# Coder-Yu/SELFRec

Hardware: AMD Instinct MI355X
Metric: train pairs/sec (XSimGCL, Yelp2018-shape) (higher is better)
Workload: dtype f32; 1 GPU; XSimGCL L=3 l*=1 eps=0.2 lambda=0.2 tau=0.2, synthetic yelp2018-shape graph (31668 users x 38048 items, 1260793 train edges), d=64, B=2048, Adam lr=1e-3; global_batch=2048, parallelism=single, bit_reproducible_step=True, launch=hipGraph replay, epoch_boundaries_in_region=1, nce_products=f32 MFMA (v_mfma_f32_16x16x4_f32)

## Files before the change

### include/selfrec_hip.h

```cpp
#ifndef SELFREC_HIP_H
#define SELFREC_HIP_H

#include <stdint.h>

#ifdef __cplusplus
extern "C" {
#endif

typedef int32_t srh_status_t;
enum {
  SRH_OK = 0,
  SRH_ERR_INVALID_ARG = -1,
  SRH_ERR_HIP = -2,
  SRH_ERR_UNSUPPORTED = -3,
  SRH_ERR_NOMEM = -4,
  SRH_ERR_STATE = -5
};

#define SRH_ABI_VERSION 31
int32_t srh_abi_version(void);
const char* srh_last_error_string(void);
int32_t srh_device_count(void);

typedef struct srh_sampler srh_sampler_t;
// ... 18 lines not shown
                                        const int32_t* h_j, const int32_t* h_uniq_u, const int32_t* h_n_uniq_u,
                                        const int32_t* h_uniq_i, const int32_t* h_n_uniq_i, int32_t user_row0,
                                        int32_t item_row0, int32_t* h_n_uniq_n, int32_t* h_seg_rows, int32_t* h_seg_end,
                                        int32_t* h_seg, int32_t* h_seg_a, int32_t* h_seg_b);
srh_status_t srh_sampler_sample_range(srh_sampler_t* s, int64_t n, int64_t k, int64_t* h_out);
srh_status_t srh_sampler_next_u32(srh_sampler_t* s, uint32_t* out);

srh_status_t srh_find_k_largest_host(int64_t k, const float* h_candidates, int64_t n, int64_t* h_out_ids,
                                     float* h_out_scores, int64_t* out_count);

srh_status_t srh_find_k_largest_host_f64(int64_t k, const double* h_candidates, int64_t n, int64_t* h_out_ids,
                                         double* h_out_scores, int64_t* out_count);

srh_status_t srh_mt19937_uniform_f32(uint32_t* h_mt624, int32_t* pos, int64_t n, float* h_out,
                                     float keep_addend, uint8_t* h_keep);

srh_status_t srh_adj_sym_normalize(int64_t n_rows, const int32_t* d_indptr,
                                   const int32_t* d_indices, const int32_t* d_edge_id,
                                   const float* d_weight, const uint8_t* d_keep,
                                   const float* d_inv_sqrt_table, int32_t table_len,
                                   float* d_deg_ws, float* d_vals, int64_t row_offset, int32_t phase,
                                   void* stream);

typedef struct srh_spmm_plan srh_spmm_plan_t;

srh_status_t srh_spmm_plan_create(srh_spmm_plan_t** out, int64_t n_rows, int64_t n_cols,
                                  const int32_t* h_indptr, int32_t split_len ,
                                  int64_t xcd_split_row, const int32_t* h_row_mid);

srh_status_t srh_spmm_plan_set_xcd_shares(srh_spmm_plan_t* plan, int32_t d, const int32_t* h_blocks_per_xcd);
int32_t srh_spmm_plan_run_tasks(const srh_spmm_plan_t* plan, int32_t d);
void srh_spmm_plan_destroy(srh_spmm_plan_t* plan);

enum { SRH_EPI_PERTURB = 1, SRH_EPI_MEAN = 2, SRH_EPI_AXPY = 4, SRH_EPI_ADAM = 8 };
#define SRH_MAX_ADAM_CLEAR 4
#define SRH_MAX_PREV 8
#define SRH_MAX_ADD 2
#define SRH_MAX_EXTRA 2

typedef struct srh_spmm_epilogue {
  int32_t flags;
  float eps;
  const float* d_noise;
  uint64_t rng_seed;
  uint64_t rng_offset;
  const int64_t* d_rng_step;
  uint64_t rng_stride;
  int32_t n_prev;
  int32_t n_add;
  const float* d_prev[SRH_MAX_PREV];
  float mean_div;
  float alpha;
  float* d_mean_out;
  const float* d_add[SRH_MAX_ADD];
  float add_scale[SRH_MAX_ADD];
  const int32_t* d_row_mark;
  const int32_t* d_col_mark;
  const int64_t* d_mark_stamp;
  const int32_t* d_add_mark;
  int32_t add_sparse_mask;
  int32_t n_extra;
  int32_t main_clean;
  float* d_extra_out[SRH_MAX_EXTRA];
  const float* d_extra_noise[SRH_MAX_EXTRA];
  uint64_t extra_rng_offset[SRH_MAX_EXTRA];
  int32_t noise_d_full;
  int32_t noise_col0;
  const float* d_row_scale;
  int32_t scale_flags;
  int32_t prev_unscale_mask;
  int32_t add_rowscale_mask;
  int32_t noise_d_valid;
  float* d_adam_param;
  float* d_adam_m;
  float* d_adam_v;
  const float* d_adam_coef;
  float adam_beta1, adam_beta2, adam_eps;
  int32_t adam_n_clear;
  const int32_t* d_adam_clear_mark;
  float* d_adam_clear[SRH_MAX_ADAM_CLEAR];
  int64_t* d_adam_cursor;
} srh_spmm_epilogue_t;
enum { SRH_SCALE_IN = 1, SRH_SCALE_OUT = 2 };

srh_status_t srh_spmm_f32(const srh_spmm_plan_t* plan, const int32_t* d_indptr,
                          const int32_t* d_indices, const float* d_vals, const float* d_x,
                          float* d_y, int32_t d, const srh_spmm_epilogue_t* epi, void* stream);

srh_status_t srh_spmm3_f32(const srh_spmm_plan_t* plan, const int32_t* d_indices, const float* d_vals0,
                           const float* d_vals1, const float* d_vals2, const float* d_x, float* d_y0,
                           float* d_y1, float* d_y2, int32_t d, void* stream);

typedef struct srh_batch_segments {
  const int32_t* d_n_uniq_u;
  const int32_t* d_n_uniq_i;
  const int32_t* d_n_uniq_n;
  const int32_t* d_seg_rows;
  const int32_t* d_seg_end;
  const int32_t* d_seg;
  const int32_t* d_seg_a;
  const int32_t* d_seg_b;
  const int32_t* d_batch_no;
  int32_t nce_rows;
  int32_t rows_are_zero;
} srh_batch_segments_t;
int64_t srh_bpr_ws_bytes(int64_t B);
srh_status_t srh_bpr_l2_fwd_bwd(const float* d_user, const float* d_item,
                                const float* d_reg_user, const float* d_reg_item,
                                const int32_t* d_u_idx, const int32_t* d_i_idx,
                                const int32_t* d_j_idx, int64_t B, const int32_t* d_n_rows,
                                int32_t d, float reg_coef, int32_t reg_include_neg,
                                float loss_scale, float* d_g_user, float* d_g_item,
                                float* d_greg_user, float* d_greg_item, double* d_losses,
                                void* d_ws, void* stream);
// ... 33 lines not shown
  int32_t g2_exclusive;
} srh_infonce_problem_t;
srh_status_t srh_infonce_fwd_bwd_multi(const srh_infonce_problem_t* problems, int32_t n_problems,
                                       int32_t d, float tau, float loss_scale, double* d_loss,
                                       void* d_ws, int32_t precision, void* stream);

#define SRH_NCE_SPLIT16 0
#define SRH_NCE_SPLIT_BF16 SRH_NCE_SPLIT16
#define SRH_NCE_F32 1
#define SRH_NCE_DEFAULT (-1)
srh_status_t srh_infonce_set_precision(int32_t mode);
int32_t srh_infonce_get_precision(void);

typedef struct srh_bpr_problem {
  const float* d_user;
  const float* d_item;
  const float* d_reg_user;
  const float* d_reg_item;
  const int32_t* d_u_idx;
  const int32_t* d_i_idx;
  const int32_t* d_j_idx;
  int64_t B;
  const int32_t* d_n_rows;
  float reg_coef;
  int32_t reg_include_neg;
  float loss_scale;
  float* d_g_user;
  float* d_g_item;
  float* d_greg_user;
  float* d_greg_item;
  double* d_losses;
  void* d_ws;
  const srh_batch_segments_t* seg;
} srh_bpr_problem_t;
srh_status_t srh_bpr_l2_fwd_bwd_p(const srh_bpr_problem_t* bpr, int32_t d, void* stream);
srh_status_t srh_bpr_infonce_fwd_bwd(const srh_bpr_problem_t* bpr, const srh_infonce_problem_t* problems,
                                     int32_t n_problems, int32_t d, float tau, float cl_scale,
                                     double* d_cl_loss, void* d_nce_ws, int32_t precision, void* stream);

srh_status_t srh_adam_step(float* d_param, const float* d_grad, float* d_m, float* d_v,
                           int64_t n_elem, int64_t step, const int64_t* d_step, float lr,
                           float beta1, float beta2, float eps, void* stream);
srh_status_t srh_adam_step_reset(float* d_param, const float* d_grad, float* d_m, float* d_v, int64_t n_rows,
                                 int32_t d, const int64_t* d_step, float lr, float beta1, float beta2, float eps,
                                 const int32_t* d_row_mark, int32_t n_clear, float* const* d_clear_tables,
                                 int64_t* d_cursor_advance, void* stream);

srh_status_t srh_score_mask_topk(const float* d_user_emb, const int32_t* d_user_ids,
                                 int64_t n_query, const float* d_item_emb, int64_t n_items,
                                 int32_t d, const int32_t* d_r_indptr, const int32_t* d_r_indices,
                                 int32_t k, float* d_scores_ws, int64_t ws_rows, int32_t* d_out_ids,
                                 float* d_out_scores, void* stream);
int64_t srh_score_mask_topk_filtered_ws_bytes(int64_t chunk_rows, int64_t sample_items, int32_t k, int32_t cap,
                                              int64_t n_items, int32_t d);
srh_status_t srh_score_mask_topk_filtered(const float* d_user_emb, const int32_t* d_user_ids, int64_t n_query,
                                          const float* d_item_emb, int64_t n_items, int32_t d,
                                          const int32_t* d_r_indptr, const int32_t* d_r_indices, int32_t k,
                                          int64_t sample_items, int32_t cap, int64_t chunk_rows, void* d_ws,
                                          int32_t* d_out_ids, float* d_out_scores, int32_t* d_out_counts,
                                          void* stream);
srh_status_t srh_topk_trim_mark_ties(const int32_t* d_ids, const float* d_scores, int64_t n_query, int32_t k1,
                                     int32_t* d_out_ids, float* d_out_scores, void* stream);
srh_status_t srh_gemm_nt_f32(const float* d_a, const float* d_b, float* d_c, int64_t m,
                             int64_t n, int32_t d, void* stream);
srh_status_t srh_topk_rows(const float* d_scores, int64_t rows, int64_t n, int32_t k,
                           int32_t* d_out_ids, float* d_out_scores, void* stream);
// ... 3 lines not shown
                                const int32_t* d_t_indices, uint8_t* d_flags, void* stream);
srh_status_t srh_metric_rows(const uint8_t* d_flags, const int32_t* d_sizes, int64_t n_query, int32_t k,
                             const int32_t* cuts, int32_t n_cuts, const double* d_gains, const double* d_ideal,
                             int32_t* d_hits, double* d_ndcg, void* stream);

srh_status_t srh_axpby(float a, const float* d_x, float b, float* d_y, int64_t n_elem, void* stream);
typedef struct {
  const int32_t* d_epoch_u;
  const int32_t* d_epoch_i;
  const int32_t* d_epoch_j;
  const int32_t* d_epoch_uniq_u;
  const int32_t* d_epoch_uniq_i;
  const int32_t* d_n_uniq_u;
  const int32_t* d_n_uniq_i;
  int64_t n_edges;
  int64_t batch_size;
  const int64_t* d_cursor;
  int32_t* d_stage_u;
  int32_t* d_stage_i;
  int32_t* d_stage_j;
  int32_t* d_stage_uniq_u;
  int32_t* d_stage_uniq_i;
  int32_t* d_meta;
  int32_t* d_row_mark;
  int32_t mark_item_offset;
  int32_t cat_item_offset;
  double* d_zero4;
  int32_t* d_stage_cat;
  int32_t* d_n_cat;
  int64_t* d_now;
  int64_t half_batches;
  float* d_adam_coef;
  float adam_lr, adam_beta1, adam_beta2;
} srh_batch_fetch_args_t;
srh_status_t srh_batch_fetch(const srh_batch_fetch_args_t* args, void* stream);
srh_status_t srh_spmm_f32_with_fetch(const srh_spmm_plan_t* plan, const int32_t* d_indptr, const int32_t* d_indices,
                                     const float* d_vals, const float* d_x, float* d_y, int32_t d,
                                     const srh_spmm_epilogue_t* epi, const srh_batch_fetch_args_t* fetch, void* stream);

srh_status_t srh_spmm_f32_probe(const srh_spmm_plan_t* plan, const int32_t* d_indices, const float* d_vals,
                                const float* d_x, float* d_y, int32_t d, const srh_spmm_epilogue_t* epi,
                                uint64_t* d_stamps, void* stream);
srh_status_t srh_spmm_gather_bound(const srh_spmm_plan_t* plan, const int32_t* d_indices, const float* d_x, float* d_scratch,
                                   int32_t d, void* stream);
srh_status_t srh_gather_floor_probe(const int32_t* d_indices, int64_t n_idx, const float* d_x, int64_t n_x_rows, int32_t d,
                                    int32_t blocks, float* d_sink, void* stream);
#define SRH_MAX_ZERO_LISTS 8
srh_status_t srh_zero_rows(int32_t n_lists, float* const* d_tables, const int32_t* const* d_idx,
                           const int32_t* const* d_counts, const int32_t* n_max,
                           const int32_t* row_offset, int32_t d,
                           int64_t* d_cursor_advance , void* stream);
srh_status_t srh_cursor_advance(int64_t* d_cursor, void* stream);

#define SRH_MAX_EXCHANGE 8
typedef struct srh_batch_lists {
  const int32_t* d_idx[5];
  const int32_t* d_count[5];
  int32_t B;
} srh_batch_lists_t;
srh_status_t srh_batch_pack(const srh_batch_lists_t* lists, int32_t n_tables, const float* const* d_tables,
                            int32_t dl, float* d_send, int32_t* d_cat_idx, int32_t* d_n_cat, void* stream);
srh_status_t srh_batch_unpack(const srh_batch_lists_t* lists, int32_t n_tables, int32_t world, int32_t dl,
                              const float* d_recv, float* const* d_compact, int32_t n_grads,
                              float* const* d_compact_grads, void* stream);
srh_status_t srh_batch_scatter(const srh_batch_lists_t* lists, int32_t n_pairs, const float* const* d_compact_grads,
                               float* const* d_local_grads, int32_t d_full, int32_t col0, int32_t dl, void* stream);
// ... 59 lines not shown
```

### selfrec_amd/_lib.py

```python
from __future__ import annotations

import ctypes as C
import os

import torch

_HERE = os.path.dirname(os.path.abspath(__file__))
LIB_PATH = os.path.join(_HERE, "lib", "libselfrec_hip.so")
ABI_VERSION = 31

SRH_EPI_PERTURB, SRH_EPI_MEAN, SRH_EPI_AXPY, SRH_EPI_ADAM = 1, 2, 4, 8
SRH_MAX_ADAM_CLEAR = 4
SRH_SCALE_IN, SRH_SCALE_OUT = 1, 2
SRH_MAX_PREV, SRH_MAX_ADD, SRH_MAX_EXTRA = 8, 2, 2


class SelfrecHipError(RuntimeError):
    pass


class BatchFetchArgs(C.Structure):
    _fields_ = [("d_epoch_u", C.c_void_p), ("d_epoch_i", C.c_void_p), ("d_epoch_j", C.c_void_p),
                ("d_epoch_uniq_u", C.c_void_p), ("d_epoch_uniq_i", C.c_void_p), ("d_n_uniq_u", C.c_void_p),
                ("d_n_uniq_i", C.c_void_p), ("n_edges", C.c_int64), ("batch_size", C.c_int64), ("d_cursor", C.c_void_p),
                ("d_stage_u", C.c_void_p), ("d_stage_i", C.c_void_p), ("d_stage_j", C.c_void_p),
                ("d_stage_uniq_u", C.c_void_p), ("d_stage_uniq_i", C.c_void_p), ("d_meta", C.c_void_p),
                ("d_row_mark", C.c_void_p), ("mark_item_offset", C.c_int32), ("cat_item_offset", C.c_int32),
                ("d_zero4", C.c_void_p), ("d_stage_cat", C.c_void_p), ("d_n_cat", C.c_void_p), ("d_now", C.c_void_p),
                ("half_batches", C.c_int64), ("d_adam_coef", C.c_void_p), ("adam_lr", C.c_float),
                ("adam_beta1", C.c_float), ("adam_beta2", C.c_float)]


class InfonceProblem(C.Structure):
    _fields_ = [("d_v1", C.c_void_p), ("d_v2", C.c_void_p), ("d_idx", C.c_void_p), ("n", C.c_int64),
                ("d_n", C.c_void_p), ("d_g1", C.c_void_p), ("d_g2", C.c_void_p), ("g2_exclusive", C.c_int32)]


class TableNceProblem(C.Structure):
    _fields_ = [("d_q", C.c_void_p), ("d_t", C.c_void_p), ("d_idx", C.c_void_p), ("B", C.c_int64), ("N", C.c_int64),
                ("loss_scale", C.c_float), ("d_loss", C.c_void_p), ("d_gq", C.c_void_p), ("d_gt", C.c_void_p)]


class L2Block(C.Structure):
    _fields_ = [("d_x", C.c_void_p), ("rows", C.c_int64), ("cols", C.c_int64), ("d_gx", C.c_void_p)]


SCALAR_WS_BYTES = 64


class BatchSegments(C.Structure):
    _fields_ = [("d_n_uniq_u", C.c_void_p), ("d_n_uniq_i", C.c_void_p), ("d_n_uniq_n", C.c_void_p),
                ("d_seg_rows", C.c_void_p), ("d_seg_end", C.c_void_p), ("d_seg", C.c_void_p), ("d_seg_a", C.c_void_p),
                ("d_seg_b", C.c_void_p), ("d_batch_no", C.c_void_p), ("nce_rows", C.c_int32), ("rows_are_zero", C.c_int32)]


class BprProblem(C.Structure):
    _fields_ = [("d_user", C.c_void_p), ("d_item", C.c_void_p), ("d_reg_user", C.c_void_p), ("d_reg_item", C.c_void_p),
                ("d_u_idx", C.c_void_p), ("d_i_idx", C.c_void_p), ("d_j_idx", C.c_void_p), ("B", C.c_int64),
                ("d_n_rows", C.c_void_p), ("reg_coef", C.c_float), ("reg_include_neg", C.c_int32),
                ("loss_scale", C.c_float), ("d_g_user", C.c_void_p), ("d_g_item", C.c_void_p),
                ("d_greg_user", C.c_void_p), ("d_greg_item", C.c_void_p), ("d_losses", C.c_void_p), ("d_ws", C.c_void_p),
                ("seg", C.POINTER(BatchSegments))]


class SpmmEpilogue(C.Structure):
    _fields_ = [
        ("flags", C.c_int32), ("eps", C.c_float), ("d_noise", C.c_void_p),
        ("rng_seed", C.c_uint64), ("rng_offset", C.c_uint64),
        ("d_rng_step", C.c_void_p), ("rng_stride", C.c_uint64),
        ("n_prev", C.c_int32), ("n_add", C.c_int32),
        ("d_prev", C.c_void_p * SRH_MAX_PREV),
        ("mean_div", C.c_float), ("alpha", C.c_float),
        ("d_mean_out", C.c_void_p),
        ("d_add", C.c_void_p * SRH_MAX_ADD),
        ("add_scale", C.c_float * SRH_MAX_ADD),
        ("d_row_mark", C.c_void_p), ("d_col_mark", C.c_void_p), ("d_mark_stamp", C.c_void_p),
        ("d_add_mark", C.c_void_p), ("add_sparse_mask", C.c_int32),
        ("n_extra", C.c_int32), ("main_clean", C.c_int32), ("d_extra_out", C.c_void_p * SRH_MAX_EXTRA),
        ("d_extra_noise", C.c_void_p * SRH_MAX_EXTRA), ("extra_rng_offset", C.c_uint64 * SRH_MAX_EXTRA),
        ("noise_d_full", C.c_int32), ("noise_col0", C.c_int32),
        ("d_row_scale", C.c_void_p), ("scale_flags", C.c_int32), ("prev_unscale_mask", C.c_int32),
        ("add_rowscale_mask", C.c_int32), ("noise_d_valid", C.c_int32),
        ("d_adam_param", C.c_void_p), ("d_adam_m", C.c_void_p), ("d_adam_v", C.c_void_p), ("d_adam_coef", C.c_void_p),
        ("adam_beta1", C.c_float), ("adam_beta2", C.c_float), ("adam_eps", C.c_float), ("adam_n_clear", C.c_int32),
        ("d_adam_clear_mark", C.c_void_p), ("d_adam_clear", C.c_void_p * SRH_MAX_ADAM_CLEAR), ("d_adam_cursor", C.c_void_p),
    ]


SRH_MAX_EXCHANGE = 8


class BatchLists(C.Structure):
    _fields_ = [("d_idx", C.c_void_p * 5), ("d_count", C.c_void_p * 5), ("B", C.c_int32)]


_vp, _i32, _i64, _f32, _u64 = C.c_void_p, C.c_int32, C.c_int64, C.c_float, C.c_uint64

SIGNATURES = {
    "srh_abi_version": (_i32, []),
    "srh_last_error_string": (C.c_char_p, []),
    "srh_device_count": (_i32, []),
    "srh_topk_trim_mark_ties": (_i32, [_vp, _vp, _i64, _i32, _vp, _vp, _vp]),
    "srh_find_k_largest_host": (_i32, [_i64, _vp, _i64, _vp, _vp, _vp]),
    "srh_find_k_largest_host_f64": (_i32, [_i64, _vp, _i64, _vp, _vp, _vp]),
    "srh_sampler_create": (_i32, [C.POINTER(_vp), _i64, _i64, _i64, _vp, _vp]),
    "srh_sampler_destroy": (None, [_vp]),
    "srh_sampler_set_state": (_i32, [_vp, _vp, _i32]),
    "srh_sampler_get_state": (_i32, [_vp, _vp, C.POINTER(_i32)]),
    "srh_sampler_seed": (_i32, [_vp, _u64]),
    "srh_sampler_shuffle": (_i32, [_vp]),
    "srh_sampler_get_order": (_i32, [_vp, _vp]),
    "srh_sampler_next_batch": (_i32, [_vp, _i64, _i64, _i32, _vp, _vp, _vp, C.POINTER(_i64)]),
    "srh_sampler_epoch": (_i32, [_vp, _i64, _i32, _vp, _vp, _vp, _vp, _vp, _vp, _vp]),
    "srh_sampler_epoch_segments": (_i32, [_vp, _i64, _vp, _vp, _vp, _vp, _vp, _vp, _vp, _i32, _i32, _vp, _vp, _vp, _vp, _vp, _vp]),
    "srh_sampler_sample_range": (_i32, [_vp, _i64, _i64, _vp]),
    "srh_sampler_next_u32": (_i32, [_vp, C.POINTER(C.c_uint32)]),
    "srh_mt19937_uniform_f32": (_i32, [_vp, C.POINTER(C.c_int32), _i64, _vp, C.c_float, _vp]),
    "srh_adj_sym_normalize": (_i32, [_i64, _vp, _vp, _vp, _vp, _vp, _vp, _i32, _vp, _vp, _i64, _i32, _vp]),
# ... 105 lines not shown
```

### selfrec_amd/csrc/common.h

```cpp
#pragma once
#include <hip/hip_runtime.h>
#include <cstdarg>
#include <cstdio>
#include <cstdint>
#include "../../include/selfrec_hip.h"

namespace srh {


void set_error(const char* fmt, ...);

#define SRH_REQUIRE(cond, ...)                    \
  do {                                            \
    if (!(cond)) {                                \
      ::srh::set_error(__VA_ARGS__);              \
      return SRH_ERR_INVALID_ARG;                 \
    }                                             \
  } while (0)

#define SRH_HIP(call)                                                              \
  do {                                                                             \
    hipError_t e_ = (call);                                                        \
    if (e_ != hipSuccess) {                                                        \
      ::srh::set_error("%s failed: %s (%s:%d)", #call, hipGetErrorString(e_),      \
// ... 23 lines not shown
__device__ __forceinline__ void batch_fetch_body(const srh_batch_fetch_args_t& f, const int block, const int n_blocks) {
  const int64_t b = f.d_cursor[0];
  const int32_t stamp = (int32_t)f.d_cursor[1];
  const int64_t bs = f.batch_size, ptr = b * bs;
  const int64_t in_epoch = ((f.half_batches > 0 && b >= f.half_batches) ? b - f.half_batches : b) * bs;
  const int64_t rows = (in_epoch >= f.n_edges) ? 0 : ((in_epoch + bs < f.n_edges) ? bs : f.n_edges - in_epoch);
  const int64_t tid = (int64_t)block * 256 + threadIdx.x, nth = (int64_t)n_blocks * 256;
  for (int64_t i = tid; i < rows; i += nth) {
    const int32_t u = f.d_epoch_u[ptr + i], p = f.d_epoch_i[ptr + i], n = f.d_epoch_j[ptr + i];
    f.d_stage_u[i] = u; f.d_stage_i[i] = p; f.d_stage_j[i] = n;
    if (f.d_row_mark) {
      f.d_row_mark[u] = stamp; f.d_row_mark[f.mark_item_offset + p] = stamp; f.d_row_mark[f.mark_item_offset + n] = stamp;
    }
  }
  int32_t a = 0, c = 0;
  if (f.d_epoch_uniq_u && rows > 0) {
    a = f.d_n_uniq_u[b];
    c = f.d_n_uniq_i[b];
    for (int64_t i = tid; i < a; i += nth) f.d_stage_uniq_u[i] = f.d_epoch_uniq_u[b * bs + i];
    for (int64_t i = tid; i < c; i += nth) f.d_stage_uniq_i[i] = f.d_epoch_uniq_i[b * bs + i];
    if (f.d_stage_cat) {
      for (int64_t i = tid; i < a; i += nth) f.d_stage_cat[i] = f.d_epoch_uniq_u[b * bs + i];
      for (int64_t i = tid; i < c; i += nth) f.d_stage_cat[a + i] = f.d_epoch_uniq_i[b * bs + i] + f.cat_item_offset;
    }
  }
  if (f.d_n_cat && tid == 0) *f.d_n_cat = a + c;
  if (f.d_zero4 && tid < 4) f.d_zero4[tid] = 0.0;
  if (f.d_now && tid < 2) f.d_now[tid] = f.d_cursor[tid];
  if (f.d_adam_coef && tid == 0) {
    const double t = (double)f.d_cursor[1];
    f.d_adam_coef[0] = (float)((double)f.adam_lr / (1.0 - pow((double)f.adam_beta1, t)));
    f.d_adam_coef[1] = (float)sqrt(1.0 - pow((double)f.adam_beta2, t));
  }
  if (tid == 0) {
    f.d_meta[0] = (int32_t)rows;
    f.d_meta[1] = a;
    f.d_meta[2] = c;
    f.d_meta[3] = (int32_t)b;
  }
}

__device__ __forceinline__ float4 f4_zero() { return make_float4(0.f, 0.f, 0.f, 0.f); }
template <bool WT>
__device__ __forceinline__ void st_f4(float4* p, float4 v) {
  if constexpr (WT) {
    typedef float fx4_t __attribute__((ext_vector_type(4)));
    const fx4_t x = {v.x, v.y, v.z, v.w};
    asm volatile("global_store_dwordx4 %0, %1, off sc1\n\ts_nop 1" ::"v"(p), "v"(x) : "memory");
  } else {
    *p = v;
  }
}
__device__ __forceinline__ void adam_element(float& m, float& v, float& p, const float g, const float b1, const float omb1,
                                             const float b2, const float omb2, const float step_size, const float bc2_sqrt,
                                             const float eps) {
#pragma clang fp contract(off)
  m = fmaf(m, b1, omb1 * g);
  v = fmaf(v, b2, omb2 * (g * g));
  p = fmaf(-step_size, m / (sqrtf(v) / bc2_sqrt + eps), p);
}
__device__ __forceinline__ float4 f4_add(float4 a, float4 b) {
  return make_float4(a.x + b.x, a.y + b.y, a.z + b.z, a.w + b.w);
}
__device__ __forceinline__ float4 f4_fma(float s, float4 x, float4 acc) {
  return make_float4(fmaf(s, x.x, acc.x), fmaf(s, x.y, acc.y), fmaf(s, x.z, acc.z), fmaf(s, x.w, acc.w));
}
__device__ __forceinline__ float4 f4_scale(float4 a, float s) {
  return make_float4(a.x * s, a.y * s, a.z * s, a.w * s);
}
__device__ __forceinline__ float f4_dot(float4 a, float4 b) {
  return fmaf(a.x, b.x, fmaf(a.y, b.y, fmaf(a.z, b.z, a.w * b.w)));
}
__device__ __forceinline__ float4 f4_shfl_xor(float4 v, int mask) {
// ... 23 lines not shown
```

### selfrec_amd/csrc/losses.hip

```cpp
#include <atomic>
#include <cstdlib>
#include <type_traits>

#include "common.h"

namespace {
using namespace srh;

typedef float floatx4 __attribute__((ext_vector_type(4)));

template <int LPR>
__device__ __forceinline__ void atomic_add_row(float* row, float4 v, int sub, float4* scr ) {
  const int lane = threadIdx.x & 63;
  scr[lane] = v;
  const float* grp = reinterpret_cast<const float*>(scr + (lane - sub));
#pragma unroll
  for (int k = 0; k < 4; ++k) unsafeAtomicAdd(row + k * LPR + sub, grp[k * LPR + sub]);
}

__device__ __forceinline__ void bpr_row(float pos, float neg, float& loss, float& coef) {
  const float x = pos - neg;
  const float sig = 1.0f / (1.0f + expf(-x));
  const float arg = 10e-6f + sig;
  loss = -logf(arg);
  coef = -(sig * (1.0f - sig)) / arg;
}

struct BprArgs {
  const float *user, *item, *reg_user, *reg_item;
  const int32_t *u_idx, *i_idx, *j_idx;
  const int32_t* d_n_rows;
  int B;
  float reg_coef, loss_scale;
  int reg_include_neg;
  float *g_user, *g_item, *greg_user, *greg_item;
  double* losses;
  double* part;
  float* coef;
  int n_blocks;
};

template <int LPR>
__device__ __forceinline__ void bpr_phase1_body(const BprArgs& a, const unsigned block_id) {
  constexpr int G = 64 / LPR;
  const int rows = a.d_n_rows ? min(*a.d_n_rows, a.B) : a.B;
  const int lane = threadIdx.x & 63, g = lane / LPR, sub = lane % LPR;
  const int b = (int)((block_id * 256u + threadIdx.x) >> 6) * G + g;
  const bool valid = b < rows;
  const int bu = valid ? a.u_idx[b] : 0, bi = valid ? a.i_idx[b] : 0, bj = valid ? a.j_idx[b] : 0;
  const float4 u = reinterpret_cast<const float4*>(a.user)[(size_t)bu * LPR + sub];
  const float4 p = reinterpret_cast<const float4*>(a.item)[(size_t)bi * LPR + sub];
  const float4 n = reinterpret_cast<const float4*>(a.item)[(size_t)bj * LPR + sub];
  const float pos = group_sum<LPR>(f4_dot(u, p));
  const float neg = group_sum<LPR>(f4_dot(u, n));
  float loss, coef;
  bpr_row(pos, neg, loss, coef);
  if (valid && sub == 0) a.coef[b] = coef;
  float4 ru = u, rp = p, rn = n;
  if (a.reg_user != a.user) ru = reinterpret_cast<const float4*>(a.reg_user)[(size_t)bu * LPR + sub];
  if (a.reg_item != a.item) {
    rp = reinterpret_cast<const float4*>(a.reg_item)[(size_t)bi * LPR + sub];
    rn = reinterpret_cast<const float4*>(a.reg_item)[(size_t)bj * LPR + sub];
  }
  double l_part = (valid && sub == 0) ? (double)loss : 0.0;
  double su = valid ? (double)f4_dot(ru, ru) : 0.0;
  double sp = valid ? (double)f4_dot(rp, rp) : 0.0;
  double sn = valid ? (double)f4_dot(rn, rn) : 0.0;
  __shared__ double s_part[4][4];
  l_part = wave_sum_d(l_part);
  su = wave_sum_d(su);
  sp = wave_sum_d(sp);
  sn = wave_sum_d(sn);
  const int wv = threadIdx.x >> 6;
  if (lane == 0) { s_part[wv][0] = l_part; s_part[wv][1] = su; s_part[wv][2] = sp; s_part[wv][3] = sn; }
  __syncthreads();
  if (threadIdx.x < 4)
    a.part[(size_t)block_id * 4 + threadIdx.x] =
        s_part[0][threadIdx.x] + s_part[1][threadIdx.x] + s_part[2][threadIdx.x] + s_part[3][threadIdx.x];
}

template <int LPR>
__device__ __forceinline__ void bpr_phase2_body(const BprArgs& a, const unsigned block_id) {
  constexpr int G = 64 / LPR;
  const int rows = a.d_n_rows ? min(*a.d_n_rows, a.B) : a.B;
  if (rows <= 0) return;
  const int lane = threadIdx.x & 63, g = lane / LPR, sub = lane % LPR;
  const int b = (int)((block_id * 256u + threadIdx.x) >> 6) * G + g;
  const int bq = min(b, rows - 1);
  const int bu = a.u_idx[bq], bi = a.i_idx[bq], bj = a.j_idx[bq];
  const float cf = a.coef[bq];
  const float4 u = reinterpret_cast<const float4*>(a.user)[(size_t)bu * LPR + sub];
  const float4 p = reinterpret_cast<const float4*>(a.item)[(size_t)bi * LPR + sub];
  const float4 n = reinterpret_cast<const float4*>(a.item)[(size_t)bj * LPR + sub];
  float4 ru = u, rp = p, rn = n;
  if (a.reg_user != a.user) ru = reinterpret_cast<const float4*>(a.reg_user)[(size_t)bu * LPR + sub];
  if (a.reg_item != a.item) {
    rp = reinterpret_cast<const float4*>(a.reg_item)[(size_t)bi * LPR + sub];
    rn = reinterpret_cast<const float4*>(a.reg_item)[(size_t)bj * LPR + sub];
  }
  __shared__ double s_tot[4];
  __shared__ float4 s_scr[4][64];
  float4* scr = s_scr[threadIdx.x >> 6];
  if (threadIdx.x < 64) {
    double t0 = 0, t1 = 0, t2 = 0, t3 = 0;
    for (int k = threadIdx.x; k < a.n_blocks; k += 64) {
      t0 += a.part[(size_t)k * 4 + 0]; t1 += a.part[(size_t)k * 4 + 1];
      t2 += a.part[(size_t)k * 4 + 2]; t3 += a.part[(size_t)k * 4 + 3];
    }
    t0 = wave_sum_d(t0); t1 = wave_sum_d(t1); t2 = wave_sum_d(t2); t3 = wave_sum_d(t3);
    if (threadIdx.x == 0) { s_tot[0] = t0; s_tot[1] = t1; s_tot[2] = t2; s_tot[3] = t3; }
  }
// ... 113 lines not shown
    acc += (double)v * (double)v;
  }
  __shared__ double s_part[4];
  acc = wave_sum_d(acc);
  if ((threadIdx.x & 63) == 0) s_part[threadIdx.x >> 6] = acc;
  __syncthreads();
  if (threadIdx.x != 0) return;
  atomicAdd(&ws->acc[k], (s_part[0] + s_part[1]) + (s_part[2] + s_part[3]));
  __threadfence();
  if (atomicAdd(&ws->ticket, 1u) != gridDim.x - 1) return;
  float emb_loss = 0.f;
  for (int j = 0; j < a.count; ++j) {
    const float nrm = (float)sqrt(atomicAdd(&ws->acc[j], 0.0));
    norms[j] = nrm;
    emb_loss += nrm / a.rows[j];
    ws->acc[j] = 0.0;
  }
  *loss = emb_loss * a.reg;
  ws->ticket = 0u;
}

__global__ __launch_bounds__(256) void l2_reg_bwd_kernel(L2Args a, const float* __restrict__ norms, const float* __restrict__ gout) {
  int k = 0;
  while (k + 1 < a.count && (int)blockIdx.x >= a.first_wg[k + 1]) ++k;
  const int wg = (int)blockIdx.x - a.first_wg[k], n_wg = a.first_wg[k + 1] - a.first_wg[k];
  const float nrm = norms[k];
  const float coef = (nrm > 0.f) ? ((gout[0] * a.reg) / a.rows[k]) / nrm : 0.f;
  const float* __restrict__ x = a.x[k];
  float* __restrict__ g = a.gx[k];
  const int64_t n = a.n[k], stride = (int64_t)n_wg * 256;
  for (int64_t i = (int64_t)wg * 256 + threadIdx.x; i < n; i += stride) g[i] = x[i] * coef;
}

constexpr int kNceSplits = 16;
constexpr float kNceKqScale = 32.0f;
constexpr float kNceInvKqScale2 = 1.0f / (kNceKqScale * kNceKqScale);
#ifndef SRH_NCE_SPLITS
#define SRH_NCE_SPLITS 8
#endif
#ifndef SRH_NCE_PV_TERMS
#define SRH_NCE_PV_TERMS 3
#endif
static_assert(SRH_NCE_SPLITS == 8 || SRH_NCE_SPLITS == 16, "SRH_NCE_SPLITS: 8 or 16");
static_assert(SRH_NCE_PV_TERMS == 3 || SRH_NCE_PV_TERMS == 6, "SRH_NCE_PV_TERMS: 3 or 6");
#ifndef SRH_NCE_WT
#define SRH_NCE_WT 1
#endif
constexpr bool kNceWT = SRH_NCE_WT != 0;
constexpr int kNceUsedSplits = SRH_NCE_SPLITS;
constexpr int kNcePvTerms = SRH_NCE_PV_TERMS;

std::atomic<int> g_nce_precision{getenv("SRH_NCE_SPLIT16") ? SRH_NCE_SPLIT16 : SRH_NCE_F32};

constexpr unsigned long long kLossUnreported = ~0ull;

struct NceWs {
  float *v1n, *v2n, *norm1, *norm2, *opart, *opart2, *lpart, *invl;
  float* ediag;
  double* losspart;
  int32_t* ticket;
  struct NcePlan* plan;
  float* etile;
  uint16_t *kq_hi[2], *kq_lo[2], *vt_hi[2], *vt_mid[2], *vt_lo[2];
  int64_t np;
  const float *src1, *src2;
  const int32_t* idx;
  const int32_t* d_n;
  int n_max;
  float *g1, *g2;
  int g2_plain;
};
constexpr int kNceMaxProblems = 4;
struct NceBatch {
  NceWs w[kNceMaxProblems];
  int count;
  int splits;
  int slots;
  int f32_only;
};

__host__ __device__ inline int64_t nce_pad(int64_t n) { return (n + 63) / 64 * 64; }

struct NcePlan {
  int n[kNceMaxProblems], per[kNceMaxProblems], splits[kNceMaxProblems], first[kNceMaxProblems + 1];
};
constexpr int kNceQueryBlock = 128, kNceKeyBlock = 32, kNceMaxPer = 128;
constexpr int kNceReuseMax = 8192;


__device__ __forceinline__ void nce_plan(const NceBatch& b, NcePlan& p) {
  int qb[kNceMaxProblems], kb[kNceMaxProblems];
  int t_min = 1;
  long long work = 0;
#pragma unroll
  for (int k = 0; k < kNceMaxProblems; ++k) {
    int n = 0;
    if (k < b.count) n = max(0, b.w[k].d_n ? min(*b.w[k].d_n, b.w[k].n_max) : b.w[k].n_max);
    p.n[k] = n;
    const int np = (int)nce_pad(n);
    qb[k] = (np + kNceQueryBlock - 1) / kNceQueryBlock;
    kb[k] = np / kNceKeyBlock;
    t_min = max(t_min, (kb[k] + kNceSplits - 1) / kNceSplits);
    work += (long long)qb[k] * kb[k];
  }
  int t = max(t_min, (int)((work + b.slots - 1) / b.slots));
  int best_t = t;
  long long best_cost = -1;
  for (int it = 0; it < 32; ++it, ++t) {
    int tasks = 0;
#pragma unroll
    for (int k = 0; k < kNceMaxProblems; ++k) tasks += qb[k] * ((kb[k] + t - 1) / t);
    const int rounds = (tasks + b.slots - 1) / b.slots;
    const long long cost = (long long)rounds * t;
    if (best_cost < 0 || cost < best_cost) { best_cost = cost; best_t = t; }
    if (rounds <= 1) break;
  }
  p.first[0] = 0;
#pragma unroll
  for (int k = 0; k < kNceMaxProblems; ++k) {
    const int sp = kb[k] > 0 ? (kb[k] + best_t - 1) / best_t : 0;
    p.splits[k] = sp;
    p.per[k] = sp > 0 ? (kb[k] + sp - 1) / sp : 0;
    p.first[k + 1] = p.first[k] + qb[k] * sp;
  }
}


inline NceWs carve_nce(void* ws, int64_t n_max, int d) {
  NceWs w;
  const int64_t np = nce_pad(n_max);
  float* p = reinterpret_cast<float*>(ws);
  w.np = np;
  w.v1n = p; p += np * d;
  w.v2n = p; p += np * d;
  w.opart = p; p += (int64_t)kNceSplits * np * d;
  w.opart2 = p; p += (int64_t)kNceSplits * np * d;
  w.norm1 = p; p += np;
  w.norm2 = p; p += np;
  w.lpart = p; p += (int64_t)kNceSplits * np;
  w.invl = p; p += np;
  w.ediag = p; p += np;
  w.losspart = reinterpret_cast<double*>(p);
  uint16_t* h = reinterpret_cast<uint16_t*>(reinterpret_cast<double*>(p) + np);
  for (int v = 0; v < 2; ++v) {
    w.kq_hi[v] = h; h += np * d;
    w.kq_lo[v] = h; h += np * d;
    w.vt_hi[v] = h; h += np * d;
    w.vt_mid[v] = h; h += np * d;
    w.vt_lo[v] = h; h += np * d;
  }
  w.ticket = reinterpret_cast<int32_t*>(h);
  w.plan = reinterpret_cast<NcePlan*>(reinterpret_cast<char*>(h) + ((4 * (np / 16 + 1) + 127) / 128) * 128);
  w.etile = np <= kNceReuseMax ? reinterpret_cast<float*>(reinterpret_cast<char*>(h) + 4 * (np / 16) + 512) : nullptr;
  return w;
}

template <int LPR>
// ... 397 lines not shown
__device__ __forceinline__ void lds_wait(floatx4 (&x)[N]) {
  static_assert(N == 4 || N == 8 || N == 16, "lds_wait: 4, 8 or 16 registers quads");
  if constexpr (N == 4) {
    asm volatile("s_waitcnt lgkmcnt(0)" : "+v"(x[0]), "+v"(x[1]), "+v"(x[2]), "+v"(x[3]));
  } else if constexpr (N == 8) {
    asm volatile("s_waitcnt lgkmcnt(0)"
                 : "+v"(x[0]), "+v"(x[1]), "+v"(x[2]), "+v"(x[3]), "+v"(x[4]), "+v"(x[5]), "+v"(x[6]), "+v"(x[7]));
  } else {
    asm volatile("s_waitcnt lgkmcnt(0)"
                 : "+v"(x[0]), "+v"(x[1]), "+v"(x[2]), "+v"(x[3]), "+v"(x[4]), "+v"(x[5]), "+v"(x[6]), "+v"(x[7]),
                   "+v"(x[8]), "+v"(x[9]), "+v"(x[10]), "+v"(x[11]), "+v"(x[12]), "+v"(x[13]), "+v"(x[14]), "+v"(x[15]));
  }
}

__device__ __forceinline__ void buffer_to_lds16(const void* base, int bytes, void* lds, int lane_off, int wave_off) {
  const __amdgpu_buffer_rsrc_t rs = __builtin_amdgcn_make_buffer_rsrc(const_cast<void*>(base), 0, bytes, 0x00020000);
  __builtin_amdgcn_raw_ptr_buffer_load_lds(rs, (__attribute__((address_space(3))) void*)lds, 16, lane_off, wave_off, 0, 0);
}

#ifdef SRH_NCEF32_STAMPS
__device__ unsigned long long g_nce_stamps[2][512 * 8 * 8];
#define SRH_STAMP(k) do { if (lane == 0) g_nce_stamps[PASS2 ? 1 : 0][((size_t)blockIdx.x * 8 + wv) * 8 + (k)] = __builtin_readcyclecounter(); } while (0)
#define SRH_STAMP_VAL(k, v) do { if (lane == 0) g_nce_stamps[PASS2 ? 1 : 0][((size_t)blockIdx.x * 8 + wv) * 8 + (k)] = (unsigned long long)(v); } while (0)
#else
#define SRH_STAMP(k) do {} while (0)
#define SRH_STAMP_VAL(k, v) do {} while (0)
#endif

__device__ __forceinline__ void st_f1_wt(float* p, float v) {
  asm volatile("global_store_dword %0, %1, off sc1" ::"v"(p), "v"(v) : "memory");
}

template <int D, bool PASS2, bool REUSE>
__global__ __launch_bounds__(512) void nce_tile_f32(NceBatch batch, float inv_tau) {
  constexpr int DQ = D / 4;
  constexpr int NT = D / 16;
  constexpr int NV = NT / 4;
  constexpr int KQ = DQ / 4;
  constexpr int RB = D * 4;
  using Cfg = NceF32<D>;
  constexpr int LPB = Cfg::kLoadsPerBlock;
  extern __shared__ __attribute__((aligned(16))) unsigned char smem[];
  float* invl_s = reinterpret_cast<float*>(smem + Cfg::kSlots * Cfg::kBlockBytes);
  const unsigned lds0 = (unsigned)(size_t)(__attribute__((address_space(3))) unsigned char*)smem;
  const int lane = threadIdx.x & 63, wv = threadIdx.x >> 6;
  SRH_STAMP(0);
  const NcePlan plan = *batch.w[0].plan;
  SRH_STAMP(1);
  const int c16 = lane & 15, g = lane >> 4;
  const int cidx = (c16 + 4) & 15;

  unsigned off_s[4], off_v[4];
#pragma unroll
  for (int t = 0; t < 4; ++t) off_s[t] = lds0 + c16 * RB + (((g + 4 * t) ^ c16) & 15) * 16;
#pragma unroll
  for (int r = 0; r < 4; ++r) off_v[r] = lds0 + (4 * g + r) * RB + ((cidx ^ (4 * g + r)) & 15) * 16;
  int ld_off[LPB];
#pragma unroll
  for (int i = 0; i < LPB; ++i) {
    const int pos = (LPB * wv + i) * 1024 + lane * 16;
    const int row = pos / RB, phys = (pos % RB) >> 4;
    ld_off[i] = row * RB + ((phys & ~15) | ((phys ^ row) & 15)) * 16;
  }

  const int n_tasks = plan.first[kNceMaxProblems];
  for (int task = blockIdx.x; task < n_tasks; task += gridDim.x) {
    int k = 0, first = 0, per = plan.per[0], splits = plan.splits[0], n = plan.n[0];
// ... 250 lines not shown
      }
      if (!wave_live) continue;
      const int key0 = kNceKeyBlock * (b0 + j);
      if constexpr (!kLogits) {
        if (key0 + kNceKeyBlock > n) reuse_step(j, std::true_type{});
        else reuse_step(j, std::false_type{});
        continue;
      }
      const bool edge = key0 + kNceKeyBlock > n || (key0 < q0 + 16 && key0 + kNceKeyBlock > q0);
      if (j + 1 < nblk) {
        if (edge) block_step(j, std::true_type{}, std::true_type{});
        else block_step(j, std::true_type{}, std::false_type{});
      } else {
        if (edge) block_step(j, std::false_type{}, std::true_type{});
        else block_step(j, std::false_type{}, std::false_type{});
      }
    }
    asm volatile("s_waitcnt vmcnt(0)" ::: "memory");
    SRH_STAMP(3);
    if (!wave_live) continue;

#pragma unroll
    for (int r = 0; r < 4; ++r)
#pragma unroll
      for (int v = 0; v < NV; ++v)
        st_f4<kNceWT>(reinterpret_cast<float4*>(opart + (size_t)(4 * g + r) * D + 4 * (cidx + 16 * v)),
                      make_float4(O[4 * v + 0][r], O[4 * v + 1][r], O[4 * v + 2][r], O[4 * v + 3][r]));
    if (!PASS2) {
      lsum += __shfl_xor(lsum, 16);
      lsum += __shfl_xor(lsum, 32);
      if (g == 0) const_cast<float*>(lpart)[(size_t)split * stride + qrow] = lsum;
    }
    SRH_STAMP(4);
  }
}

template <int LPR>
__device__ __forceinline__ void nce_finish_both_body(const NceBatch& batch, const NceFinishArgs& a, const unsigned bx,
                                                     const unsigned bz) {
  constexpr int G = 64 / LPR;
  const NceWs& w = batch.w[bz];
  const int n = w.d_n ? min(*w.d_n, w.n_max) : w.n_max;
  const int wave = (int)((bx * 256u + threadIdx.x) >> 6);
  const int n_waves = (int)(w.np / G);
  if (n <= 0 || wave >= n_waves) return;
  const int lane = threadIdx.x & 63, g = lane / LPR, sub = lane % LPR;
  __shared__ float4 s_scr[4][64];
  int splits = batch.splits;
  if (batch.slots > 0) {
    splits = batch.w[0].plan->splits[bz];
  }
  const double part = wave_sum_d(nce_finish_row<LPR>(w, a, n, wave * G + g, sub, s_scr[threadIdx.x >> 6], splits));
  __shared__ double wg_part[4];
  if (lane == 0) wg_part[threadIdx.x >> 6] = part;
  __syncthreads();
  const int n_wgs = n_waves / 4;
  if (threadIdx.x < 64) {
    if (lane == 0) store_f64_sc1(w.losspart + bx, (wg_part[0] + wg_part[1]) + (wg_part[2] + wg_part[3]));
    asm volatile("s_waitcnt vmcnt(0)" ::: "memory");
    int ticket = 0;
    if (lane == 0) ticket = __hip_atomic_fetch_add(w.ticket, 1, __ATOMIC_RELAXED, __HIP_MEMORY_SCOPE_AGENT);
    ticket = __builtin_amdgcn_readfirstlane(ticket);
    if (ticket == n_wgs - 1) {
      __builtin_amdgcn_fence(__ATOMIC_ACQUIRE, "agent");
      if (lane == 0) __hip_atomic_store(w.ticket, 0, __ATOMIC_RELAXED, __HIP_MEMORY_SCOPE_AGENT);
      double t = 0.0;
// ... 205 lines not shown
        }
        if (__builtin_amdgcn_ballot_w64(missing) == 0) break;
        __builtin_amdgcn_s_sleep(1);
      }
#pragma unroll
      for (int q = 0; q < 8; ++q) t += __builtin_bit_cast(double, v[q]);
    }
    t = wave_sum_d(t);
    s_li[k] = n > 0 ? (double)fa.loss_scale * t / (double)n : 0.0;
  }
  __syncthreads();
  if (threadIdx.x == 0) {
    double t = 0.0;
    for (int j = 0; j < batch.count; ++j) t += s_li[j];
    atomicAdd(fa.loss, t);
  }
}

template <int LPR, bool ZERO>
__global__ __launch_bounds__(256) void rows_finish(NceBatch batch, NceFinishArgs fa, BprArgs bpr, SegArgs sg) {
  rows_finish_body<LPR, ZERO>(batch, fa, bpr, sg);
}
template <int LPR>
void launch_rows_finish(const NceBatch& batch, const NceFinishArgs& fa, const BprArgs& bp, const SegArgs& sg, hipStream_t st) {
  constexpr int G = 64 / LPR;
  const int grid = (3 * bp.B + 4 * G - 1) / (4 * G);
  if (sg.rows_are_zero) rows_finish<LPR, true><<<grid, 256, 0, st>>>(batch, fa, bp, sg);
  else rows_finish<LPR, false><<<grid, 256, 0, st>>>(batch, fa, bp, sg);
}

template <int D>
srh_status_t launch_infonce(const srh_infonce_problem_t* pr, int count, float tau, float loss_scale, double* loss,
                            void* ws, hipStream_t st, int precision, const BprArgs* bpr = nullptr,
                            const SegArgs* seg = nullptr) {
  constexpr int LPR = D / 4, G = 64 / LPR;
  NceBatch batch{};
  batch.count = count;
  batch.splits = kNceUsedSplits;
  int np_max = 0;
  char* cursor = reinterpret_cast<char*>(ws);
  for (int k = 0; k < count; ++k) {
    NceWs w = carve_nce(cursor, pr[k].n, D);
    cursor += srh_infonce_ws_bytes(pr[k].n, D);
    w.src1 = pr[k].d_v1; w.src2 = pr[k].d_v2; w.idx = pr[k].d_idx; w.d_n = pr[k].d_n; w.n_max = (int)pr[k].n;
    w.g1 = pr[k].d_g1; w.g2 = pr[k].d_g2;
    w.g2_plain = pr[k].g2_exclusive != 0 && pr[k].d_g2 != pr[k].d_g1;
    batch.w[k] = w;
    np_max = std::max(np_max, (int)w.np);
  }
  const float inv_tau = 1.0f / tau;
  const bool f32 = precision == SRH_NCE_F32;
  int grid_f32 = 0;
  if (f32) {
    if constexpr (D > 128) {
      srh::set_error("infonce_fwd_bwd: the all-f32 MFMA path serves d = 64 / 128");
      return SRH_ERR_UNSUPPORTED;
    }
    int64_t most = 0;
    for (int k = 0; k < count; ++k) {
      if (batch.w[k].np / kNceKeyBlock > (int64_t)kNceSplits * kNceMaxPer) {
        srh::set_error("infonce_fwd_bwd: the all-f32 MFMA path serves n <= %d", kNceSplits * kNceMaxPer * kNceKeyBlock);
        return SRH_ERR_UNSUPPORTED;
      }
      most += (batch.w[k].np + kNceQueryBlock - 1) / kNceQueryBlock * kNceSplits;
    }
    batch.slots = srh::cu_count();
    batch.f32_only = 1;
    grid_f32 = (int)std::min<int64_t>(batch.slots, most);
  }
  dim3 gp((np_max / G + 3) / 4, 2, count);
  BprArgs bp{};
  int n_bpr = 0;
  if (bpr) {
    bp = *bpr;
    n_bpr = bp.n_blocks = ((bp.B + G - 1) / G + 3) / 4;
    nce_prep_bpr1<LPR><<<n_bpr + (int)(gp.x * 2 * count), 256, 0, st>>>(batch, bp, n_bpr, (int)gp.x);
  } else {
    nce_prep<LPR><<<gp, 256, 0, st>>>(batch);
  }
  SRH_LAUNCH_CHECK();
  NceFinishArgs fa{inv_tau, loss_scale, loss};
  dim3 fb((np_max / G + 3) / 4, 1, count);
  if (!f32) {
    constexpr int kLds = nce_lds_bytes<D, kNcePvTerms>();
    static const bool attr_set = [] {
      (void)hipFuncSetAttribute((const void*)nce_tile_lds<D, false, 1, 8, kNcePvTerms>, hipFuncAttributeMaxDynamicSharedMemorySize, kLds);
      (void)hipFuncSetAttribute((const void*)nce_tile_lds<D, true, 1, 8, kNcePvTerms>, hipFuncAttributeMaxDynamicSharedMemorySize, kLds);
      return true;
    }();
    (void)attr_set;
    dim3 gl((np_max + 127) / 128, batch.splits, count);
    nce_tile_lds<D, false, 1, 8, kNcePvTerms><<<gl, 512, kLds, st>>>(batch, inv_tau);
    SRH_LAUNCH_CHECK();
    nce_tile_lds<D, true, 1, 8, kNcePvTerms><<<gl, 512, kLds, st>>>(batch, inv_tau);
    SRH_LAUNCH_CHECK();
  } else if constexpr (D <= 128) {
    constexpr int kLds = NceF32<D>::kLds;
    static const bool attr_set = [] {
      (void)hipFuncSetAttribute((const void*)nce_tile_f32<D, false, false>, hipFuncAttributeMaxDynamicSharedMemorySize, kLds);
      (void)hipFuncSetAttribute((const void*)nce_tile_f32<D, true, false>, hipFuncAttributeMaxDynamicSharedMemorySize, kLds);
      (void)hipFuncSetAttribute((const void*)nce_tile_f32<D, false, true>, hipFuncAttributeMaxDynamicSharedMemorySize, kLds);
      (void)hipFuncSetAttribute((const void*)nce_tile_f32<D, true, true>, hipFuncAttributeMaxDynamicSharedMemorySize, kLds);
      return true;
    }();
    (void)attr_set;
    bool reuse = true;
    for (int k = 0; k < count; ++k) reuse = reuse && batch.w[k].etile != nullptr;
    if (reuse) {
      nce_tile_f32<D, false, true><<<grid_f32, 512, kLds, st>>>(batch, inv_tau);
      SRH_LAUNCH_CHECK();
      nce_tile_f32<D, true, true><<<grid_f32, 512, kLds, st>>>(batch, inv_tau);
    } else {
      nce_tile_f32<D, false, false><<<grid_f32, 512, kLds, st>>>(batch, inv_tau);
      SRH_LAUNCH_CHECK();
      nce_tile_f32<D, true, false><<<grid_f32, 512, kLds, st>>>(batch, inv_tau);
    }
    SRH_LAUNCH_CHECK();
  }
  if (bpr && seg) {
    for (int k = 0; k < count; ++k)
      SRH_REQUIRE(batch.w[k].np >= (3 * bp.B + 4 * G - 1) / (4 * G),
                  "bpr_infonce_fwd_bwd: with batch segments every InfoNCE problem must be sized for the batch (n >= ~3 B d / 256)");
    launch_rows_finish<LPR>(batch, fa, bp, *seg, st);
  }
  else if (bpr) nce_finish_bpr2<LPR><<<n_bpr + (int)(fb.x * count), 256, 0, st>>>(batch, fa, bp, n_bpr, (int)fb.x);
  else nce_finish_both<LPR><<<fb, 256, 0, st>>>(batch, fa);
  SRH_LAUNCH_CHECK();
  return SRH_OK;
}

template <int LPR>
srh_status_t launch_bpr(const BprArgs& a, hipStream_t st, const SegArgs* seg = nullptr) {
  constexpr int G = 64 / LPR;
  const int blocks = ((a.B + G - 1) / G + 3) / 4;
  BprArgs b = a;
  b.n_blocks = blocks;
  bpr_phase1<LPR><<<blocks, 256, 0, st>>>(b);
  SRH_LAUNCH_CHECK();
  if (seg) {
    NceBatch none{};
    launch_rows_finish<LPR>(none, NceFinishArgs{}, b, *seg, st);
  } else {
    bpr_phase2<LPR><<<blocks, 256, 0, st>>>(b);
  }
  SRH_LAUNCH_CHECK();
  return SRH_OK;
}

// ... 101 lines not shown
}

srh_status_t srh_l2_reg_fwd(const srh_l2_block_t* blocks, int32_t n_blocks, float reg, void* d_scalar_ws,
                            float* d_norms, float* d_loss, void* stream) {
  SRH_REQUIRE(d_scalar_ws && d_norms && d_loss, "l2_reg_fwd: null argument");
  L2Args a{};
  if (srh_status_t s = l2_args(blocks, n_blocks, reg, false, a)) return s;
  l2_reg_fwd_kernel<<<a.first_wg[n_blocks], 256, 0, srh::as_stream(stream)>>>(a, reinterpret_cast<ScalarWs*>(d_scalar_ws),
                                                                             d_norms, d_loss);
  SRH_LAUNCH_CHECK();
  return SRH_OK;
}

srh_status_t srh_l2_reg_bwd(const srh_l2_block_t* blocks, int32_t n_blocks, float reg, const float* d_norms,
                            const float* d_gout, void* stream) {
  SRH_REQUIRE(d_norms && d_gout, "l2_reg_bwd: null argument");
  L2Args a{};
  if (srh_status_t s = l2_args(blocks, n_blocks, reg, true, a)) return s;
  l2_reg_bwd_kernel<<<a.first_wg[n_blocks], 256, 0, srh::as_stream(stream)>>>(a, d_norms, d_gout);
  SRH_LAUNCH_CHECK();
  return SRH_OK;
}

int64_t srh_infonce_ws_bytes(int64_t n, int32_t d) {
  if (n <= 0 || d <= 0) return 0;
  const int64_t np = nce_pad(n);
  return 4 * (2 * np * d + 2 * (int64_t)kNceSplits * np * d + 4 * np + (int64_t)kNceSplits * np) + 8 * np +
         20 * np * d + 4 * (np / 16) + 512 +
         (np <= kNceReuseMax ? 4 * np * np : 0);
}

static srh_status_t infonce_entry(const srh_infonce_problem_t* problems, int32_t n_problems, int32_t d, float tau,
                                  float loss_scale, double* d_loss, void* d_ws, int32_t precision, void* stream,
                                  const BprArgs* bpr, const SegArgs* seg = nullptr) {
  SRH_REQUIRE(precision == SRH_NCE_DEFAULT || precision == SRH_NCE_SPLIT16 || precision == SRH_NCE_F32,
              "infonce_fwd_bwd: unknown precision %d", precision);
  if (precision == SRH_NCE_DEFAULT) {
    precision = g_nce_precision.load(std::memory_order_relaxed);
    if (d == 256 && precision == SRH_NCE_F32) {
      static std::atomic<bool> said{false};
      if (!said.exchange(true))
        fprintf(stderr, "[selfrec_hip] infonce: d = 256 has no all-f32 MFMA path; SRH_NCE_DEFAULT resolves to SRH_NCE_SPLIT16 "
                        "(f16 hi+lo / bf16 hi+mid operands, f32 accumulation: logits to 2^-22) for these calls\n");
      precision = SRH_NCE_SPLIT16;
    }
  }
  SRH_REQUIRE(problems && d_loss && d_ws, "infonce_fwd_bwd: null argument");
  SRH_REQUIRE(n_problems >= 1 && n_problems <= kNceMaxProblems, "infonce_fwd_bwd: 1..%d problems per call", kNceMaxProblems);
  SRH_REQUIRE(d == 64 || d == 128 || d == 256, "infonce_fwd_bwd: d=%d unsupported (need 64, 128 or 256)", d);
  SRH_REQUIRE(d != 256 || precision != SRH_NCE_F32,
              "infonce_fwd_bwd: the all-f32 MFMA path serves d = 64 / 128 (d = 256: the split path only)");
  for (int k = 0; k < n_problems; ++k) {
    const srh_infonce_problem_t& p = problems[k];
    SRH_REQUIRE(p.d_v1 && p.d_v2 && p.d_g1 && p.d_g2, "infonce_fwd_bwd: null tensor in problem %d", k);
    SRH_REQUIRE(p.n > 0 && p.n < (int64_t(1) << 24), "infonce_fwd_bwd: bad n in problem %d", k);
  }
  if (!(tau >= 0.03f)) {
    srh::set_error("infonce_fwd_bwd: temperature %g below 0.03 needs a running max (not implemented)", (double)tau);
    return SRH_ERR_UNSUPPORTED;
  }
  hipStream_t st = srh::as_stream(stream);
  if (d == 64) return launch_infonce<64>(problems, n_problems, tau, loss_scale, d_loss, d_ws, st, precision, bpr, seg);
  if (d == 128) return launch_infonce<128>(problems, n_problems, tau, loss_scale, d_loss, d_ws, st, precision, bpr, seg);
  return launch_infonce<256>(problems, n_problems, tau, loss_scale, d_loss, d_ws, st, precision, bpr, seg);
}

#ifdef SRH_NCEF32_STAMPS
srh_status_t srh_debug_nce_stamps(unsigned long long* h_out ) {
  SRH_HIP(hipDeviceSynchronize());
  SRH_HIP(hipMemcpyFromSymbol(h_out, HIP_SYMBOL(g_nce_stamps), sizeof(g_nce_stamps)));
  return SRH_OK;
}
#endif

srh_status_t srh_infonce_set_precision(int32_t mode) {
  SRH_REQUIRE(mode == SRH_NCE_SPLIT_BF16 || mode == SRH_NCE_F32, "infonce_set_precision: unknown mode %d", mode);
  g_nce_precision.store(mode, std::memory_order_relaxed);
  return SRH_OK;
}
int32_t srh_infonce_get_precision(void) { return g_nce_precision.load(std::memory_order_relaxed); }

srh_status_t srh_infonce_fwd_bwd_multi(const srh_infonce_problem_t* problems, int32_t n_problems, int32_t d,
                                       float tau, float loss_scale, double* d_loss, void* d_ws, int32_t precision,
                                       void* stream) {
  return infonce_entry(problems, n_problems, d, tau, loss_scale, d_loss, d_ws, precision, stream, nullptr);
}

srh_status_t srh_bpr_infonce_fwd_bwd(const srh_bpr_problem_t* b, const srh_infonce_problem_t* problems,
                                     int32_t n_problems, int32_t d, float tau, float cl_scale, double* d_cl_loss,
                                     void* d_nce_ws, int32_t precision, void* stream) {
  SRH_REQUIRE(b, "bpr_infonce_fwd_bwd: null bpr problem");
  SRH_REQUIRE(b->d_user && b->d_item && b->d_reg_user && b->d_reg_item && b->d_u_idx && b->d_i_idx && b->d_j_idx,
              "bpr_infonce_fwd_bwd: null input");
  SRH_REQUIRE(b->d_g_user && b->d_g_item && b->d_greg_user && b->d_greg_item && b->d_losses && b->d_ws,
              "bpr_infonce_fwd_bwd: null output");
  SRH_REQUIRE(b->B > 0 && b->B < (int64_t(1) << 30), "bpr_infonce_fwd_bwd: bad batch size");
  BprArgs a{b->d_user, b->d_item, b->d_reg_user, b->d_reg_item, b->d_u_idx, b->d_i_idx, b->d_j_idx, b->d_n_rows,
            (int)b->B, b->reg_coef, b->loss_scale, b->reg_include_neg, b->d_g_user, b->d_g_item, b->d_greg_user,
            b->d_greg_item, b->d_losses, reinterpret_cast<double*>(b->d_ws),
            reinterpret_cast<float*>(reinterpret_cast<char*>(b->d_ws) + bpr_part_bytes(b->B)), 0};
  SegArgs sg{};
  if (b->seg)
    if (srh_status_t st = seg_args(b->seg, n_problems, sg)) return st;
  return infonce_entry(problems, n_problems, d, tau, cl_scale, d_cl_loss, d_nce_ws, precision, stream, &a, b->seg ? &sg : nullptr);
}

srh_status_t srh_bpr_l2_fwd_bwd_p(const srh_bpr_problem_t* b, int32_t d, void* stream) {
  SRH_REQUIRE(b, "bpr_l2_fwd_bwd_p: null bpr problem");
  SRH_REQUIRE(b->d_user && b->d_item && b->d_reg_user && b->d_reg_item && b->d_u_idx && b->d_i_idx && b->d_j_idx,
              "bpr_l2_fwd_bwd_p: null input");
  SRH_REQUIRE(b->d_g_user && b->d_g_item && b->d_greg_user && b->d_greg_item && b->d_losses && b->d_ws,
              "bpr_l2_fwd_bwd_p: null output");
  SRH_REQUIRE(b->B > 0 && b->B < (int64_t(1) << 28), "bpr_l2_fwd_bwd_p: bad batch size");
  SRH_REQUIRE(srh::dim_supported(d), "bpr_l2_fwd_bwd_p: d=%d unsupported", d);
  BprArgs a{b->d_user, b->d_item, b->d_reg_user, b->d_reg_item, b->d_u_idx, b->d_i_idx, b->d_j_idx, b->d_n_rows,
            (int)b->B, b->reg_coef, b->loss_scale, b->reg_include_neg, b->d_g_user, b->d_g_item, b->d_greg_user,
            b->d_greg_item, b->d_losses, reinterpret_cast<double*>(b->d_ws),
            reinterpret_cast<float*>(reinterpret_cast<char*>(b->d_ws) + bpr_part_bytes(b->B)), 0};
  SegArgs sg{};
  if (b->seg)
    if (srh_status_t st = seg_args(b->seg, 0, sg)) return st;
  hipStream_t st = srh::as_stream(stream);
  const SegArgs* sp = b->seg ? &sg : nullptr;
  switch (d) {
    case 32: return launch_bpr<8>(a, st, sp);
    case 64: return launch_bpr<16>(a, st, sp);
    case 128: return launch_bpr<32>(a, st, sp);
    default: return launch_bpr<64>(a, st, sp);
  }
}

srh_status_t srh_infonce_fwd_bwd(const float* d_v1, const float* d_v2, const int32_t* d_idx, int64_t n,
                                 const int32_t* d_n, int32_t d, float tau, float loss_scale, double* d_loss,
                                 float* d_g1, float* d_g2, void* d_ws, void* stream) {
  srh_infonce_problem_t p{d_v1, d_v2, d_idx, n, d_n, d_g1, d_g2};
  return srh_infonce_fwd_bwd_multi(&p, 1, d, tau, loss_scale, d_loss, d_ws, SRH_NCE_DEFAULT, stream);
}
// ... 3 lines not shown
```

### selfrec_amd/csrc/spmm.hip

```cpp
#include <algorithm>
#include <cstdlib>
#include <new>
#include <vector>

#include "common.h"

#ifndef SRH_Y_WT
#define SRH_Y_WT 1
#endif

namespace {

using namespace srh;
constexpr bool kYWT = SRH_Y_WT != 0;

struct Seg {
  int32_t row, start, end, slot;
};
struct Heavy {
  int32_t row, first_slot, n_slots, pad;
};

struct DevEpilogue {
  int32_t flags;
  float eps;
  const float* noise;
  uint32_t seed_lo, seed_hi, off_lo, off_hi;
  const int64_t* rng_step;
  uint64_t rng_stride;
  float alpha;
  int32_t n_prev, n_add;
  const float* prev[SRH_MAX_PREV];
  float mean_rcp;
  float* mean_out;
  const float* add[SRH_MAX_ADD];
  float add_scale[SRH_MAX_ADD];
  const int32_t* row_mark;
  const int32_t* col_mark;
  const int64_t* mark_stamp;
  const int32_t* add_mark;
  int32_t add_sparse;
  int32_t n_extra, main_clean;
  float* extra_out[SRH_MAX_EXTRA];
  const float* extra_noise[SRH_MAX_EXTRA];
  uint32_t extra_off_lo[SRH_MAX_EXTRA], extra_off_hi[SRH_MAX_EXTRA];
  int32_t noise_d_full, noise_col0;
  int32_t noise_d_valid;
  const float* row_scale;
  int32_t scale_flags, prev_unscale, add_rowscale;
  unsigned long long* stamps;
  float4 *adam_p, *adam_m, *adam_v;
  const float* adam_coef;
  float adam_b1, adam_b2, adam_eps;
  int32_t adam_n_clear;
  const int32_t* adam_clear_mark;
  float4* adam_clear[SRH_MAX_ADAM_CLEAR];
  int64_t* adam_cursor;
};

__device__ __forceinline__ uint32_t lowbias32(uint32_t x) {
  x ^= x >> 16; x *= 0x7feb352dU; x ^= x >> 15; x *= 0x846ca68bU; x ^= x >> 16;
  return x;
}
__device__ __forceinline__ uint4 counter_rng4(uint64_t ctr, uint32_t sub, uint32_t seed_lo, uint32_t seed_hi) {
  const uint32_t key = lowbias32((uint32_t)ctr ^ seed_lo) + lowbias32((uint32_t)(ctr >> 32) ^ seed_hi);
  const uint32_t base = key + sub * 0x9E3779B1U;
  return make_uint4(lowbias32(base), lowbias32(base + 0x85EBCA6BU), lowbias32(base + 0xC2B2AE35U),
                    lowbias32(base + 0x27D4EB2FU));
}
__device__ __forceinline__ float u01(uint32_t x) { return (float)(x >> 8) * (1.0f / 16777216.0f); }

__device__ __forceinline__ float4 sum_partials_agent(const float4* base, int t0, int step, int hn, int stride4) {
  typedef float fx4 __attribute__((ext_vector_type(4)));
  float4 sum = f4_zero();
  int t = t0;
  for (; t + 7 * step < hn; t += 8 * step) {
    fx4 p[8];
#pragma unroll
    for (int k = 0; k < 8; ++k)
      asm volatile("global_load_dwordx4 %0, %1, off sc1" : "=v"(p[k]) : "v"(base + (size_t)(t + k * step) * stride4) : "memory");
    asm volatile("s_waitcnt vmcnt(0)"
                 : "+v"(p[0]), "+v"(p[1]), "+v"(p[2]), "+v"(p[3]), "+v"(p[4]), "+v"(p[5]), "+v"(p[6]), "+v"(p[7])::"memory");
#pragma unroll
    for (int k = 0; k < 8; ++k) sum = f4_add(sum, make_float4(p[k].x, p[k].y, p[k].z, p[k].w));
  }
  for (; t < hn; t += step) {
    fx4 q;
    asm volatile("global_load_dwordx4 %0, %1, off sc1\n\ts_waitcnt vmcnt(0)" : "=v"(q) : "v"(base + (size_t)t * stride4) : "memory");
    sum = f4_add(sum, make_float4(q.x, q.y, q.z, q.w));
  }
// ... 20 lines not shown
      float4 z;
      if (noise) {
        z = nr[q];
      } else {
        const uint4 r = counter_rng4(ctr, (uint32_t)q, ep.seed_lo, ep.seed_hi);
        z = make_float4(u01(r.x), u01(r.y), u01(r.z), u01(r.w));
      }
      return padded ? mask_valid(z, q, ep.noise_d_valid) : z;
    };
    ss = 0.f;
    for (int q = sub; q < nq; q += LPR) { const float4 z = draw(q); ss += f4_dot(z, z); }
    ss = group_sum<LPR>(ss);
    nu = draw(own);
  } else {
    if (noise) {
      nu = reinterpret_cast<const float4*>(noise)[at];
    } else {
      uint64_t ctr = (((uint64_t)off_hi << 32) | off_lo) + (uint64_t)row;
      if (ep.rng_step) ctr += (uint64_t)(*ep.rng_step) * ep.rng_stride;
      uint4 r = counter_rng4(ctr, (uint32_t)sub, ep.seed_lo, ep.seed_hi);
      nu = make_float4(u01(r.x), u01(r.y), u01(r.z), u01(r.w));
    }
    if (ep.noise_d_valid < 4 * LPR) nu = mask_valid(nu, sub, ep.noise_d_valid);
    ss = group_sum<LPR>(f4_dot(nu, nu));
  }
  const float scale = ep.eps / fmaxf(sqrtf(ss), 1e-12f);
  y.x += sgnf(y.x) * (nu.x * scale);
  y.y += sgnf(y.y) * (nu.y * scale);
  y.z += sgnf(y.z) * (nu.z * scale);
  y.w += sgnf(y.w) * (nu.w * scale);
  return y;
}

template <int LPR, bool ADAM = false>
__device__ __forceinline__ void row_epilogue(float4 y, int row, int sub, bool store, float4* __restrict__ Y,
                                             const DevEpilogue& ep, const float r = 1.0f) {
  if (!store) return;
  const size_t at = (size_t)row * LPR + sub;
  float4 mm, vv, pp;
  if constexpr (ADAM) {
    mm = ep.adam_m[at]; vv = ep.adam_v[at]; pp = ep.adam_p[at];
  }
  if (ep.scale_flags & SRH_SCALE_IN) y = f4_scale(y, r);
  if (ep.flags & SRH_EPI_AXPY) {
    y = f4_scale(y, ep.alpha);
    const bool marked = !ep.add_mark || ep.add_mark[row] == (int)(*ep.mark_stamp);
    for (int t = 0; t < ep.n_add; ++t) {
      if (((ep.add_sparse >> t) & 1) && !marked) continue;
      float4 a = reinterpret_cast<const float4*>(ep.add[t])[at];
      const float sc = ((ep.add_rowscale >> t) & 1) ? ep.add_scale[t] * r : ep.add_scale[t];
      y = f4_fma(sc, a, y);
    }
  }
  if constexpr (ADAM) {
    const float step_size = ep.adam_coef[0], bc2_sqrt = ep.adam_coef[1];
    const float b1 = ep.adam_b1, b2 = ep.adam_b2, omb1 = 1.0f - b1, omb2 = 1.0f - b2, aeps = ep.adam_eps;
#define SRH_ADAM_LANE(c) adam_element(mm.c, vv.c, pp.c, y.c, b1, omb1, b2, omb2, step_size, bc2_sqrt, aeps);
    SRH_ADAM_LANE(x) SRH_ADAM_LANE(y) SRH_ADAM_LANE(z) SRH_ADAM_LANE(w)
#undef SRH_ADAM_LANE
    st_f4<kYWT>(ep.adam_m + at, mm); st_f4<kYWT>(ep.adam_v + at, vv); st_f4<kYWT>(ep.adam_p + at, pp);
    if (ep.adam_n_clear > 0 && ep.adam_clear_mark[row] == (int)(*ep.mark_stamp)) {
      for (int k = 0; k < ep.adam_n_clear; ++k) ep.adam_clear[k][at] = f4_zero();
    }
    return;
  }
  const bool out_scaled = (ep.scale_flags & SRH_SCALE_OUT) != 0;
  if (ep.flags & SRH_EPI_PERTURB) {
    const float4 raw = y;
    if (!ep.main_clean) y = perturb_row<LPR>(raw, row, sub, at, ep.noise, ep.off_lo, ep.off_hi, ep);
    for (int k = 0; k < ep.n_extra; ++k) {
      const float4 yk = perturb_row<LPR>(raw, row, sub, at, ep.extra_noise[k], ep.extra_off_lo[k], ep.extra_off_hi[k], ep);
      if (store) st_f4<kYWT>(reinterpret_cast<float4*>(ep.extra_out[k]) + at, out_scaled ? f4_scale(yk, r) : yk);
    }
  }
  if (store) st_f4<kYWT>(Y + at, out_scaled ? f4_scale(y, r) : y);
  if (ep.flags & SRH_EPI_MEAN) {
    const float rinv = (ep.prev_unscale && r > 0.f) ? 1.0f / r : 0.f;
    float4 m = y;
    if (ep.n_prev > 0) {
      m = reinterpret_cast<const float4*>(ep.prev[0])[at];
      if (ep.prev_unscale & 1) m = f4_scale(m, rinv);
      for (int t = 1; t < ep.n_prev; ++t) {
        float4 pt = reinterpret_cast<const float4*>(ep.prev[t])[at];
        if ((ep.prev_unscale >> t) & 1) pt = f4_scale(pt, rinv);
        m = f4_add(m, pt);
      }
      m = f4_add(m, y);
    }
    if (store) {
      float4 o = f4_scale(m, ep.mean_rcp);
      st_f4<kYWT>(reinterpret_cast<float4*>(ep.mean_out) + at, o);
    }
  }
}

typedef float floatx4_t __attribute__((ext_vector_type(4)));

struct Task {
  int32_t kind, first, count, pad;
};
constexpr int kShortRow = 64;

template <int K>
__device__ __forceinline__ int row_bcast_i(int x) { return __builtin_amdgcn_update_dpp(0, x, 0x150 + K, 0xf, 0xf, false); }
template <int K>
__device__ __forceinline__ float row_bcast_f(float x) { return __int_as_float(row_bcast_i<K>(__float_as_int(x))); }

template <int LPR>
__device__ __forceinline__ float4 ld_x(const float4* __restrict__ X, int c, int sub) {
  const unsigned off = (unsigned)c * (unsigned)(LPR * 16) + (unsigned)(sub * 16);
  return *reinterpret_cast<const float4*>(reinterpret_cast<const char*>(X) + off);
}

__device__ __forceinline__ void store_f4_sc1(float4* p, float4 v) {
  floatx4_t x = {v.x, v.y, v.z, v.w};
  asm volatile("global_store_dwordx4 %0, %1, off sc1\n\ts_nop 1" ::"v"(p), "v"(x) : "memory");
}

typedef float floatx2_t __attribute__((ext_vector_type(2)));
struct Acc2 { floatx2_t lo, hi; };

#define SRH_DPP_OR(T)                                                                                          \
  asm volatile("v_or_b32_dpp %0, %1, %2 row_newbcast:" #T " row_mask:0xf bank_mask:0xf" : "=v"(off[T & 7]) : "v"(cs), "v"(sub16))
#define SRH_DPP_MOV(T)                                                                                         \
  asm volatile("v_mov_b32_dpp %0, %1 row_newbcast:" #T " row_mask:0xf bank_mask:0xf" : "=v"(vv[T & 7]) : "v"(v))
// ... 84 lines not shown
#pragma unroll
  for (int t = 0; t < 4; ++t) {
    xx[t] = f4_zero();
    if (vv[t] != 0.f) xx[t] = ld_x<LPR>(X, cc[t], sub);
  }
#pragma unroll
  for (int t = 0; t < 4; ++t) acc = f4_fma(vv[t], xx[t], acc);
}

template <int LPR>
__device__ __forceinline__ void gather16_compact(int c, float v, const float4* __restrict__ X, int sub, float4& acc) {
  const int lane = threadIdx.x & 63, e16 = lane & 15, row0 = lane & 48;
  const bool alive = v != 0.f;
  const unsigned long long bal = __ballot(alive);
  if (bal == 0ull) return;
  const unsigned gm = (unsigned)(bal >> row0) & 0xffffu;
  const int n_g = __popc(gm), before = __popc(gm & ((1u << e16) - 1u));
  const int dst = row0 + (alive ? before : n_g + (e16 - before));
  c = __builtin_amdgcn_ds_permute(dst << 2, c);
  v = __int_as_float(__builtin_amdgcn_ds_permute(dst << 2, __float_as_int(v)));
  const int nmax = max(max(__popcll(bal & 0xffffull), __popcll((bal >> 16) & 0xffffull)),
                       max(__popcll((bal >> 32) & 0xffffull), __popcll(bal >> 48)));
  gather4_live<LPR, 0>(c, v, X, sub, acc);
  if (nmax > 4) gather4_live<LPR, 4>(c, v, X, sub, acc);
  if (nmax > 8) gather4_live<LPR, 8>(c, v, X, sub, acc);
  if (nmax > 12) gather4_live<LPR, 12>(c, v, X, sub, acc);
}

struct alignas(64) Task64 {
  int32_t kind, count, slot, pad;
  int32_t row[4], start[4], end[4];
};

template <int LPR, bool COLMASK, bool PROBE = false, bool LATEPF = false, bool FLOOR = false, bool ADAM = false>
__global__ __launch_bounds__(256) __attribute__((amdgpu_waves_per_eu(8, 8))) void spmm_rows_kernel(const Task64* __restrict__ tasks, int n_tasks,
                                                        const int32_t* __restrict__ indices,
                                                        const float* __restrict__ vals,
                                                        const float4* __restrict__ X, float4* __restrict__ Y,
                                                        float4* __restrict__ partial,
                                                        const Heavy* __restrict__ heavy,
                                                        const int32_t* __restrict__ slot_owner,
                                                        int32_t* __restrict__ tickets, DevEpilogue ep,
                                                        const int n_fetch, const srh_batch_fetch_args_t rider) {
  constexpr int G = 64 / LPR;
  constexpr int CH = 16 * G;
  if ((int)blockIdx.x < n_fetch) {
    srh::batch_fetch_body(rider, (int)blockIdx.x, n_fetch);
    return;
  }
  const int wave = __builtin_amdgcn_readfirstlane((int)(((blockIdx.x - n_fetch) * 256u + threadIdx.x) >> 6));
  if (wave >= n_tasks) return;
  const int lane = threadIdx.x & 63;
  if constexpr (ADAM) {
    if (ep.adam_cursor && wave == 0 && lane == 0) { ep.adam_cursor[0] += 1; ep.adam_cursor[1] += 1; }
  }
  unsigned long long t_begin = 0;
  unsigned xcc = 0;
  if constexpr (PROBE) {
    t_begin = wall_clock64();
    asm volatile("s_getreg_b32 %0, hwreg(HW_REG_XCC_ID)" : "=s"(xcc));
  }
  auto leave = [&]() {
    if constexpr (PROBE) if (lane == 0) {
      ep.stamps[3 * (size_t)wave] = t_begin;
      ep.stamps[3 * (size_t)wave + 1] = wall_clock64();
      ep.stamps[3 * (size_t)wave + 2] = xcc & 0xfu;
    }
  };
  const int g = lane / LPR, sub = lane % LPR, e16 = lane & 15;
  const unsigned sub16 = (unsigned)sub * 16u;
  const int stamp = ep.mark_stamp ? (int)(*ep.mark_stamp) : 0;
  const floatx4_t zero = {0.f, 0.f, 0.f, 0.f};
  Acc2 acc = {{0.f, 0.f}, {0.f, 0.f}};
  floatx4_t xx[8];
#pragma unroll
  for (int t = 0; t < 8; ++t) xx[t] = zero;

  const Task64* tp = tasks + wave;
  const int kind = tp->kind, count = tp->count, slot = tp->slot;
  int row = tp->row[0], s = tp->start[0], e = tp->end[0];
// ... 61 lines not shown
    const int slot = lane_slot(coop_rounds(e - base));
    return slot < 0 ? e : base + G * slot + g;
  };
  auto short_at = [&](int q, int maxlen_) {
    const int slot = lane_slot(maxlen_ - 16 * q);
    return slot < 0 ? e : s + 16 * q + slot;
  };
  auto total = [&]() { return COLMASK ? accm : make_float4(acc.lo.x, acc.lo.y, acc.hi.x, acc.hi.y); };

  if (kind == 0) {
    row = __builtin_amdgcn_readfirstlane(row); s = __builtin_amdgcn_readfirstlane(s); e = __builtin_amdgcn_readfirstlane(e);
    if (ep.row_mark && ep.row_mark[row] != stamp) { leave(); return; }
    const float r = ep.row_scale ? ep.row_scale[row] : 1.0f;
    fetch(coop_at(s), e, cs, v);
    if (LATE) {
      for (int base = s; base < e; base += CH) chunk_late(coop_rounds(e - base), coop_at(base + CH), e);
    } else
    for (int base = s; base < e; base += CH) {
      const bool more = base + CH < e;
      if (prefetch && more) fetch(coop_at(base + CH), e, csn, vn);
      chunk(coop_rounds(e - base));
      if (prefetch) { cs = csn; v = vn; }
      else if (more) fetch(coop_at(base + CH), e, cs, v);
    }
    float4 a4 = total();
    if constexpr (FLOOR) {
      if (a4.x == 123456.789f) Y[0] = a4;
      leave();
      return;
    }
#pragma unroll
    for (int m = LPR; m < 64; m <<= 1) a4 = f4_add(a4, f4_shfl_xor(a4, m));
    if (slot < 0) {
      row_epilogue<LPR, ADAM>(a4, row, sub, g == 0, Y, ep, r);
      leave();
      return;
    }
    if (g == 0) store_f4_sc1(partial + (size_t)slot * LPR + sub, a4);
    const int hid = __builtin_amdgcn_readfirstlane(slot_owner[slot]);
    const Heavy h = heavy[hid];
    const int hfirst = __builtin_amdgcn_readfirstlane(h.first_slot);
    const int hn = __builtin_amdgcn_readfirstlane(h.n_slots);
    asm volatile("s_waitcnt vmcnt(0)" ::: "memory");
    int ticket = 0;
    if (lane == 0) ticket = __hip_atomic_fetch_add(tickets + hid, 1, __ATOMIC_RELAXED, __HIP_MEMORY_SCOPE_AGENT);
    ticket = __builtin_amdgcn_readfirstlane(ticket);
    if (ticket != hn - 1) { leave(); return; }
    if (lane == 0) __hip_atomic_store(tickets + hid, 0, __ATOMIC_RELAXED, __HIP_MEMORY_SCOPE_AGENT);
    float4 sum = sum_partials_agent(partial + (size_t)hfirst * LPR + sub, g, G, hn, LPR);
#pragma unroll
    for (int m = LPR; m < 64; m <<= 1) sum = f4_add(sum, f4_shfl_xor(sum, m));
    row_epilogue<LPR, ADAM>(sum, row, sub, g == 0, Y, ep, r);
    leave();
    return;
  }

  const bool live = g < count && (!ep.row_mark || ep.row_mark[row] == stamp);
  if (ep.row_mark && __ballot(live) == 0ull) { leave(); return; }
  const float r = ep.row_scale ? ep.row_scale[row] : 1.0f;
  if (!live) e = s;
  int maxlen = e - s;
#pragma unroll
  for (int m = LPR; m < 64; m <<= 1) maxlen = max(maxlen, __shfl_xor(maxlen, m));
  maxlen = __builtin_amdgcn_readfirstlane(maxlen);
  fetch(short_at(0, maxlen), e, cs, v);
  if (LATE) {
    for (int q = 0; q * 16 < maxlen; ++q) chunk_late(maxlen - 16 * q, short_at(q + 1, maxlen), e);
  } else
  for (int q = 0; q * 16 < maxlen; ++q) {
    const bool more = (q + 1) * 16 < maxlen;
    if (prefetch && more) fetch(short_at(q + 1, maxlen), e, csn, vn);
    chunk(maxlen - 16 * q);
    if (prefetch) { cs = csn; v = vn; }
    else if (more) fetch(short_at(q + 1, maxlen), e, cs, v);
  }
  if constexpr (FLOOR) {
    const float4 a4 = total();
    if (a4.x == 123456.789f) Y[0] = a4;
  } else {
    row_epilogue<LPR, ADAM>(total(), row, sub, live, Y, ep, r);
  }
  leave();
}

template <int LPR, int T0>
__device__ __forceinline__ void gather8x3(int c, float v0, float v1, float v2, const float4* __restrict__ X, int sub,
                                          float4 (&acc)[3]) {
  int cc[8];
  float a0[8], a1[8], a2[8];
  float4 xx[8];
#define SRH_BC(T) cc[T] = row_bcast_i<T0 + T>(c); a0[T] = row_bcast_f<T0 + T>(v0); a1[T] = row_bcast_f<T0 + T>(v1); \
  a2[T] = row_bcast_f<T0 + T>(v2);
  SRH_BC(0) SRH_BC(1) SRH_BC(2) SRH_BC(3) SRH_BC(4) SRH_BC(5) SRH_BC(6) SRH_BC(7)
#undef SRH_BC
#pragma unroll
  for (int t = 0; t < 8; ++t) {
    xx[t] = f4_zero();
    if (a0[t] != 0.f) xx[t] = ld_x<LPR>(X, cc[t], sub);
  }
#pragma unroll
  for (int t = 0; t < 8; ++t) {
    acc[0] = f4_fma(a0[t], xx[t], acc[0]);
    acc[1] = f4_fma(a1[t], xx[t], acc[1]);
    acc[2] = f4_fma(a2[t], xx[t], acc[2]);
  }
}

template <int LPR>
__global__ __launch_bounds__(256) void spmm_rows3_kernel(const Task* __restrict__ tasks, int n_tasks,
                                                         const Seg* __restrict__ segs,
                                                         const int32_t* __restrict__ indices,
                                                         const float* __restrict__ vals0, const float* __restrict__ vals1,
                                                         const float* __restrict__ vals2, const float4* __restrict__ X,
// ... 496 lines not shown
#pragma unroll
      for (int t = 0; t < 8; ++t) nxt[t] = idx[nb + t * G + g];
    }
    float4 x[8];
#pragma unroll
    for (int t = 0; t < 8; ++t) x[t] = ld_x<LPR>(X, cur[t], sub);
#pragma unroll
    for (int t = 0; t < 8; ++t) acc = f4_add(acc, x[t]);
  }
  if (acc.x == 123.456f) sink[0] = acc;
}

}

struct srh_spmm_plan {
  int64_t n_rows = 0, n_cols = 0, nnz = 0;
  int32_t n_heavy = 0, n_slots = 0, split_len = 0;
  int32_t n_tasks[5] = {0, 0, 0, 0, 0};
  Task* d_tasks[5] = {nullptr, nullptr, nullptr, nullptr, nullptr};
  Seg* d_tsegs = nullptr;
  Task64* d_tasks64[5] = {nullptr, nullptr, nullptr, nullptr, nullptr};
  std::vector<Task64> h_tasks64[5];
  int32_t n_run[5] = {0, 0, 0, 0, 0};
  size_t cap64[5] = {0, 0, 0, 0, 0};
  Heavy* d_heavy = nullptr;
  int32_t* d_slot_owner = nullptr;
  int32_t* d_tickets = nullptr;
  float* d_partial = nullptr;
};

static srh_status_t translate_epilogue(const srh_spmm_epilogue_t* epi, int32_t d, const float* d_x, const float* d_y,
                                       DevEpilogue& ep) {
  if (epi) {
    SRH_REQUIRE((epi->flags & ~(SRH_EPI_PERTURB | SRH_EPI_MEAN | SRH_EPI_AXPY | SRH_EPI_ADAM)) == 0,
                "spmm_f32: unknown epilogue flag");
    ep.flags = epi->flags;
    ep.eps = epi->eps;
    ep.noise = epi->d_noise;
    ep.seed_lo = (uint32_t)epi->rng_seed; ep.seed_hi = (uint32_t)(epi->rng_seed >> 32);
    ep.off_lo = (uint32_t)epi->rng_offset; ep.off_hi = (uint32_t)(epi->rng_offset >> 32);
    ep.rng_step = epi->d_rng_step;
    ep.rng_stride = epi->rng_stride;
    ep.row_mark = epi->d_row_mark;
    ep.col_mark = epi->d_col_mark;
    ep.mark_stamp = epi->d_mark_stamp;
    ep.add_mark = epi->d_add_mark;
    ep.add_sparse = epi->add_sparse_mask;
    if (epi->d_row_scale || epi->scale_flags || epi->prev_unscale_mask || epi->add_rowscale_mask) {
      SRH_REQUIRE(epi->d_row_scale && d >= 64, "spmm_f32: row scaling needs d_row_scale and d >= 64");
      SRH_REQUIRE((epi->scale_flags & ~(SRH_SCALE_IN | SRH_SCALE_OUT)) == 0, "spmm_f32: unknown scale flag");
      ep.row_scale = epi->d_row_scale;
      ep.scale_flags = epi->scale_flags;
      ep.prev_unscale = epi->prev_unscale_mask;
      ep.add_rowscale = epi->add_rowscale_mask;
    }
    if (epi->noise_d_full) {
      SRH_REQUIRE(epi->noise_d_full % 32 == 0 && epi->noise_col0 >= 0 && epi->noise_col0 % d == 0 &&
                      epi->noise_col0 + d <= epi->noise_d_full,
                  "spmm_f32: column slice [%d, %d) of %d-wide rows is not supported (aligned slices of rows a multiple of 32 wide)",
                  epi->noise_col0, epi->noise_col0 + d, epi->noise_d_full);
      ep.noise_d_full = epi->noise_d_full;
      ep.noise_col0 = epi->noise_col0;
    }
    if (epi->n_extra || epi->main_clean) {
      SRH_REQUIRE((epi->flags & SRH_EPI_PERTURB) && !(epi->flags & SRH_EPI_MEAN) && epi->n_extra >= 0 &&
                      epi->n_extra <= SRH_MAX_EXTRA,
                  "spmm_f32: extra perturbed outputs need PERTURB without MEAN and at most %d of them", SRH_MAX_EXTRA);
// ... 24 lines not shown
      SRH_REQUIRE(epi->n_add >= 0 && epi->n_add <= SRH_MAX_ADD, "spmm_f32: bad AXPY epilogue");
      ep.n_add = epi->n_add;
      ep.alpha = epi->alpha;
      for (int t = 0; t < epi->n_add; ++t) {
        SRH_REQUIRE(epi->d_add[t], "spmm_f32: null add[%d]", t);
        ep.add[t] = epi->d_add[t];
        ep.add_scale[t] = epi->add_scale[t];
      }
    }
  }
  if (epi && (epi->flags & SRH_EPI_ADAM)) {
    SRH_REQUIRE(d >= 64 && !(epi->flags & (SRH_EPI_PERTURB | SRH_EPI_MEAN)) && !(epi->scale_flags & SRH_SCALE_OUT) &&
                    !epi->d_row_mark && !epi->noise_d_full,
                "spmm_f32: ADAM runs on whole rows of >= 64 columns, after AXPY only (no PERTURB / MEAN / SCALE_OUT / row marks)");
    SRH_REQUIRE(epi->d_adam_param && epi->d_adam_m && epi->d_adam_v && epi->d_adam_coef, "spmm_f32: ADAM: null table");
    SRH_REQUIRE(epi->d_adam_param != d_x && epi->d_adam_m != d_x && epi->d_adam_v != d_x, "spmm_f32: ADAM updates a table the product reads");
    SRH_REQUIRE(epi->adam_n_clear >= 0 && epi->adam_n_clear <= SRH_MAX_ADAM_CLEAR &&
                    (epi->adam_n_clear == 0 || (epi->d_adam_clear_mark && epi->d_mark_stamp)),
                "spmm_f32: ADAM: at most %d tables to clear, with their row marks and the stamp", SRH_MAX_ADAM_CLEAR);
    SRH_REQUIRE(!epi->d_adam_cursor || (epi->d_mark_stamp != epi->d_adam_cursor && epi->d_mark_stamp != epi->d_adam_cursor + 1),
                "spmm_f32: ADAM: d_mark_stamp must be a copy of the step when the launch advances the cursor");
    ep.adam_p = reinterpret_cast<float4*>(epi->d_adam_param);
    ep.adam_m = reinterpret_cast<float4*>(epi->d_adam_m);
    ep.adam_v = reinterpret_cast<float4*>(epi->d_adam_v);
    ep.adam_coef = epi->d_adam_coef;
    ep.adam_b1 = epi->adam_beta1; ep.adam_b2 = epi->adam_beta2; ep.adam_eps = epi->adam_eps;
    ep.adam_n_clear = epi->adam_n_clear;
    ep.adam_clear_mark = epi->d_adam_clear_mark;
    for (int k = 0; k < epi->adam_n_clear; ++k) {
      SRH_REQUIRE(epi->d_adam_clear[k] && epi->d_adam_clear[k] != d_x, "spmm_f32: ADAM: table %d to clear is null or the product's x", k);
      ep.adam_clear[k] = reinterpret_cast<float4*>(epi->d_adam_clear[k]);
    }
    ep.adam_cursor = epi->d_adam_cursor;
  }
  if (!ep.noise_d_full) { ep.noise_d_full = d; ep.noise_col0 = 0; }
  ep.noise_d_valid = ep.noise_d_full;
  if (epi && epi->noise_d_valid) {
    SRH_REQUIRE(epi->noise_d_valid > 0 && epi->noise_d_valid <= ep.noise_d_full,
                "spmm_f32: noise_d_valid = %d outside (0, %d]", epi->noise_d_valid, ep.noise_d_full);
    SRH_REQUIRE(d >= 64 || epi->noise_d_valid == ep.noise_d_full,
                "spmm_f32: zero-padded rows (noise_d_valid < row width) are served on tables of >= 64 columns, not %d", d);
    ep.noise_d_valid = epi->noise_d_valid;
  }
  SRH_REQUIRE(d > 32 || ep.noise_d_full % 32 == 0 || !(ep.flags & SRH_EPI_PERTURB),
              "spmm_f32: PERTURB on %d-wide rows needs the whole row width (a multiple of 32) in noise_d_full", d);
  return SRH_OK;
}

extern "C" {

srh_status_t srh_spmm_plan_create(srh_spmm_plan_t** out, int64_t n_rows, int64_t n_cols,
                                  const int32_t* h_indptr, int32_t split_len, int64_t xcd_split_row,
                                  const int32_t* h_row_mid) {
  SRH_REQUIRE(out && h_indptr, "spmm_plan_create: null argument");
  SRH_REQUIRE(n_rows > 0 && n_cols > 0, "spmm_plan_create: bad shape");
  SRH_REQUIRE(n_rows < (int64_t(1) << 31) && n_cols < (int64_t(1) << 31), "spmm_plan_create: shape exceeds int32");
  if (split_len <= 0) split_len = 512;
  SRH_REQUIRE(split_len % 64 == 0, "spmm_plan_create: split_len must be a multiple of 64");
  SRH_REQUIRE(h_indptr[0] == 0, "spmm_plan_create: indptr[0] != 0");
  SRH_REQUIRE(xcd_split_row >= 0 && xcd_split_row <= n_rows, "spmm_plan_create: xcd_split_row out of range");
  struct ClsSeg { Seg seg; int8_t half; };
  std::vector<ClsSeg> segs;
  std::vector<Heavy> heavy;
  std::vector<int32_t> slot_owner;
  segs.reserve((size_t)n_rows + 1024);
  int32_t n_slots = 0;
// ... 246 lines not shown
    for (int k = 0; k < 8; ++k) depth = std::max(depth, q[k].size());
    list.assign(depth * 8 * 4, empty);
    for (int k = 0; k < 8; ++k)
      for (size_t pos = 0; pos < q[k].size(); ++pos)
        for (int w = 0; w < 4; ++w) list[(pos * 8 + k) * 4 + w] = block(q[k][pos], w);
  }
  if (list.size() > plan->cap64[gi]) {
    Task64* fresh = nullptr;
    hipError_t err = hipMalloc(&fresh, sizeof(Task64) * list.size());
    if (err != hipSuccess) { srh::set_error("spmm_plan_set_xcd_shares: %s", hipGetErrorString(err)); return SRH_ERR_HIP; }
    (void)hipFree(plan->d_tasks64[gi]);
    plan->d_tasks64[gi] = fresh;
    plan->cap64[gi] = list.size();
  }
  hipError_t err = hipDeviceSynchronize();
  if (err == hipSuccess && !list.empty())
    err = hipMemcpy(plan->d_tasks64[gi], list.data(), sizeof(Task64) * list.size(), hipMemcpyHostToDevice);
  if (err != hipSuccess) { srh::set_error("spmm_plan_set_xcd_shares: %s", hipGetErrorString(err)); return SRH_ERR_HIP; }
  plan->n_run[gi] = (int32_t)list.size();
  return SRH_OK;
}

static srh_status_t spmm_launch(const srh_spmm_plan_t* plan, const int32_t* d_indices, const float* d_vals, const float* d_x,
                                float* d_y, int32_t d, const srh_spmm_epilogue_t* epi, const srh_batch_fetch_args_t* fetch,
                                unsigned long long* d_stamps, void* stream, bool floor_only) {
  srh_batch_fetch_args_t fetch_args{};
  int n_fetch = 0;
  if (fetch) {
    SRH_REQUIRE(d >= 64 && !(epi && (epi->d_col_mark || epi->d_row_mark)),
                "spmm_f32_with_fetch: d >= 64, and the product must not depend on the batch's marks");
    if (srh_status_t rc = srh::check_fetch_args(fetch, fetch_args)) return rc;
    n_fetch = srh::kFetchBlocks;
  }
  SRH_REQUIRE(plan && d_indices && d_x && d_y, "spmm_f32: null argument");
  SRH_REQUIRE(d_vals || (d >= 64 && !(epi && epi->d_col_mark)),
              "spmm_f32: a pattern matrix (d_vals == NULL) needs d >= 64 and no column marks");
  SRH_REQUIRE(srh::dim_supported(d) || d == 8 || d == 16, "spmm_f32: d=%d unsupported (need 8, 16, 32, 64, 128 or 256)", d);
  SRH_REQUIRE(d_x != d_y, "spmm_f32: x and y must not alias");
  SRH_REQUIRE(plan->n_cols * (int64_t)d * 4 < (int64_t(1) << 32), "spmm_f32: x (%lld rows x %d) must be smaller than 4 GiB",
              (long long)plan->n_cols, d);
  DevEpilogue ep{};
  if (srh_status_t rc = translate_epilogue(epi, d, d_x, d_y, ep)) return rc;
  hipStream_t st = srh::as_stream(stream);
#define SRH_LAUNCH(KERNEL, GI, XT, YT)                                                                              \
  KERNEL<<<(plan->n_tasks[GI] + 3) / 4, 256, 0, st>>>(plan->d_tasks[GI], plan->n_tasks[GI], plan->d_tsegs, d_indices,  \
                                                      d_vals, reinterpret_cast<const XT*>(d_x), reinterpret_cast<YT*>(d_y), \
                                                      reinterpret_cast<YT*>(plan->d_partial), plan->d_heavy,          \
                                                      plan->d_slot_owner, plan->d_tickets, ep)
  switch (d) {
    case 8: SRH_LAUNCH(spmm_pair_kernel, 0, float, float); break;
    case 16: SRH_LAUNCH(spmm_slice_kernel<4>, 4, float4, float4); break;
    case 32: SRH_LAUNCH(spmm_slice_kernel<8>, 0, float4, float4); break;
    default: {
      SRH_REQUIRE(plan->n_cols * (int64_t)d * 4 < (int64_t(1) << 31), "spmm_f32: x (%lld rows x %d) must be smaller than 2 GiB",
                  (long long)plan->n_cols, d);
#define SRH_LAUNCH_ROWS(LPRV, GI, CM, PR, ...)                                                                       \
  spmm_rows_kernel<LPRV, CM, PR, ##__VA_ARGS__><<<(plan->n_run[GI] + 3) / 4 + n_fetch, 256, 0, st>>>(           \
      plan->d_tasks64[GI], plan->n_run[GI], d_indices, d_vals, reinterpret_cast<const float4*>(d_x),                \
      reinterpret_cast<float4*>(d_y), reinterpret_cast<float4*>(plan->d_partial), plan->d_heavy, plan->d_slot_owner, \
      plan->d_tickets, ep, n_fetch, fetch_args)
      ep.stamps = d_stamps;
      SRH_REQUIRE(!(ep.flags & SRH_EPI_ADAM) || !(floor_only || d_stamps || ep.col_mark),
                  "spmm_f32: ADAM runs on the plain launch (no column marks, not under the probes)");
      if (floor_only) {
        if (d == 64) SRH_LAUNCH_ROWS(16, 1, false, false, false, true);
        else if (d == 128) SRH_LAUNCH_ROWS(32, 2, false, false, false, true);
        else SRH_LAUNCH_ROWS(64, 3, false, false, false, true);
      } else if (d_stamps) {
        SRH_REQUIRE(!ep.col_mark, "spmm_f32_probe: no column marks");
        if (d == 64) SRH_LAUNCH_ROWS(16, 1, false, true);
        else if (d == 128) SRH_LAUNCH_ROWS(32, 2, false, true);
        else SRH_LAUNCH_ROWS(64, 3, false, true);
      } else if (ep.col_mark) {
        if (d == 64) SRH_LAUNCH_ROWS(16, 1, true, false);
        else if (d == 128) SRH_LAUNCH_ROWS(32, 2, true, false);
        else SRH_LAUNCH_ROWS(64, 3, true, false);
      } else if (ep.flags & SRH_EPI_ADAM) {
        if (d == 64) SRH_LAUNCH_ROWS(16, 1, false, false, false, false, true);
        else if (d == 128) SRH_LAUNCH_ROWS(32, 2, false, false, false, false, true);
        else SRH_LAUNCH_ROWS(64, 3, false, false, false, false, true);
      } else if (ep.row_mark && d == 64) {
        SRH_LAUNCH_ROWS(16, 1, false, false, true);
      } else {
        if (d == 64) SRH_LAUNCH_ROWS(16, 1, false, false);
        else if (d == 128) SRH_LAUNCH_ROWS(32, 2, false, false);
        else SRH_LAUNCH_ROWS(64, 3, false, false);
      }
#undef SRH_LAUNCH_ROWS
    }
  }
#undef SRH_LAUNCH
  SRH_LAUNCH_CHECK();
  return SRH_OK;
}

}
```

### selfrec_amd/engine.py

```python
from __future__ import annotations

import os
import threading

import numpy as np
import torch
import torch.distributed as _dist

from . import layouts, ops
from ._lib import SelfrecHipError
from .comm import AbiComm, TorchComm, TwoHopRows, default_comm, shard_adjacency
from .layouts import SLICE_WIDTHS, parse_grid

MODELS = ("MF", "LightGCN", "XSimGCL", "SimGCL", "SGL")


class FusedTrainer:
    reuse_epoch_arrays = True

    def __init__(self, data, emb_size, *, model, n_layers=2, lr=1e-3, reg=1e-4, cl_rate=0.2, eps=0.2,
                 tau=0.2, layer_cl=1, drop_rate=0.1, aug_type=1, batch_size=2048, user_emb=None, item_emb=None,
                 noise_fn=None, rng_seed=0x5E1F0EC, use_graph=False, device=None, shard=False, comm=None,
                 nce_precision=None, sampler_seed=None):
        if model not in MODELS:
            raise SelfrecHipError(f"FusedTrainer: unknown model {model!r}")
        ops.require_gpu()
        self.model, self.data = model, data
        self.d_valid = int(emb_size)
        widths = ops.NCE_WIDTHS if model in ("XSimGCL", "SimGCL", "SGL") else ops.ROW_WIDTHS
        self.d = ops.padded_width(self.d_valid, widths) if self.d_valid > 0 else None
        if self.d is None:
            raise SelfrecHipError(f"{model}: embedding.size = {emb_size} -- the fused kernels serve up to {widths[-1]} columns"
                                  + (" (InfoNCE; the op-level tier, selfrec_amd.dropin, takes wider rows)" if widths[-1] < 256 else ""))
        self.L = 0 if model == "MF" else int(n_layers)
        self.lr, self.reg, self.cl_rate, self.eps, self.tau = float(lr), float(reg), float(cl_rate), float(eps), float(tau)
        if model == "SimGCL":
            self.tau = 0.2
        self.layer_cl, self.drop_rate, self.aug_type = int(layer_cl), float(drop_rate), int(aug_type)
        self.B = int(batch_size)
        self.noise_fn = noise_fn
        if nce_precision is not None and nce_precision not in ops.NCE_PRECISIONS:
            raise SelfrecHipError(f"FusedTrainer: nce_precision {nce_precision!r}: one of {sorted(ops.NCE_PRECISIONS)} or None")
# ... 71 lines not shown
        self.use_marks = True
        self.sparse_reset = True
        self.views = []
        if model in ("SimGCL", "SGL"):
            for _ in range(2):
                self.views.append({"F": buf(), "Y": [buf() for _ in range(self.L)], "gF": buf()})
        self.view_adj = [None, None]
        self._view_vals = [torch.empty_like(self.adj.vals), torch.empty_like(self.adj.vals)] if model == "SGL" else None
        self.losses = torch.zeros(4, dtype=torch.float64, device=dev)
        self.stage = {k: torch.zeros(B, dtype=torch.int32, device=dev) for k in ("u", "i", "j", "uniq_u", "uniq_i")}
        self.stage_cat = torch.zeros(2 * B, dtype=torch.int32, device=dev)
        self.meta = torch.zeros(4, dtype=torch.int32, device=dev)
        self.cursor = torch.tensor([0, 1], dtype=torch.int64, device=dev)
        self.now = self.cursor.clone()
        single = dev.type == "cuda" and self.place.single_gpu_step
        self.fused_reset = single
        self.vfree = (single and self.L >= 2 and self.d >= 64
                      and model in ("LightGCN", "XSimGCL", "SimGCL") and self.graph.weight is None)
        self.dinv = self.graph.dinv if self.vfree else None
        self.adj_cm = None
        if single and self.L >= 1 and self.d >= 64:
            self.adj_cm = self.adj.replanned(split_len=256)
        self.ride_fetch = single and self.L >= 2 and self.d >= 64 and model in ("LightGCN", "XSimGCL", "SimGCL")
        self.adam_coef = torch.zeros(2, dtype=torch.float32, device=dev)
        self.fuse_adam = (single and not self.sync.active and self.sparse_reset and self.L >= 2 and self.w >= 64
                          and model != "MF" and tuple(self.m.shape) == tuple(self.E0.shape)
                          and getattr(ops, "ADAM_EPILOGUE", False) and os.environ.get("SRH_FUSE_ADAM", "1") != "0")
        self.n_cat = torch.zeros(1, dtype=torch.int32, device=dev)
        self.bpr_ws = ops.bpr_ws(B, dev)
        self.nce_ws = None
        if model in ("XSimGCL", "SimGCL", "SGL"):
            one = ops.infonce_ws(2 * B if model == "SGL" else B, d, dev)
            self.nce_ws = torch.empty(one.numel() * (1 if model == "SGL" else 2), dtype=torch.uint8, device=dev)
        E = self.sampler.n_edges
        self.epoch_batches = (E + B - 1) // B
        nb = self.epoch_batches
        self._epoch_slot = {"u": nb * B, "i": nb * B, "j": nb * B, "uniq_u": nb * B, "uniq_i": nb * B,
                            "n_uniq_u": nb, "n_uniq_i": nb}
        if self.det_scatter:
            self._epoch_slot.update({"n_uniq_n": nb, "seg_rows": 3 * nb * B, "seg_end": 3 * nb * B, "seg": 3 * nb * B,
                                     "seg_a": 3 * nb * B, "seg_b": nb * B})
        self._epoch_dev = {k: torch.zeros(2 * n, dtype=torch.int32, device=dev) for k, n in self._epoch_slot.items()}
        self._live_half = None
        self._half_free = [None, None]
        self._copy_stream = None
        self._pinned = [None, None]
        self._stage_pending = [None, None]
        self._hip_lock = threading.RLock()
        self._epoch_ready = False
        self.step_count = 0
        self.use_graph = bool(use_graph) and self.place.graph_by_default(os.environ.get("SRH_SHARDED_GRAPH"))
        self._graph = None
        self._noise_call = 0
        self._rng_calls = max(16, 2 * self.L)
        self.colx.init_exchange(self)
        self.xcd_shares = self._calibrate_xcd_shares()

    def _calibrate_xcd_shares(self, rounds=5):
        self.xcd_calibration = None
        if not layouts.calibration_enabled() or self.dev.type != "cuda" or not self.place.single_gpu_step:
            return None
        if self.L < 1 or self.d != 64:
            return None
        done = self.adj.__dict__.setdefault("_xcd_calibrated", {})
        key = self.d
        if key in done:
# ... 204 lines not shown
            self._half_free[self._live_half] = ev
        if self.place.replicated_batches:
            w3 = np.arange(1, 4, dtype=np.int64)
            self._assert_replicated("the sampled epoch (u, i, j streams)",
                                    [int(host[k].astype(np.int64).sum()) for k in ("u", "i", "j")] +
                                    [int((host[k][:3 * (host[k].size // 3)].astype(np.int64).reshape(-1, 3) * w3).sum())
                                     for k in ("u", "i", "j")])
        self._epoch_host = host
        self._epoch_ready = True
        self._live_half = half
        self.cursor[0:1].fill_(half * self.epoch_batches)

    def begin_epoch(self):
        self.upload_epoch(self.sample_epoch_host())
        return self.epoch_batches

    def _noise(self):
        if self.noise_fn is None:
            return None
        t = torch.as_tensor(self.noise_fn((self.N, self.d_valid)), dtype=torch.float32)
        if self.d_valid != self.d:
            t = torch.nn.functional.pad(t, (0, self.d - self.d_valid))
        return self.rows.place_noise(t.to(self.dev), self.d)

    def _rng_offset(self, call):
        return (call * self.P + self.rows.rng_row_offset()) & ((1 << 62) - 1)

    def _slice_kw(self):
        kw = self.colx.slice_kw()
        if self.d_valid != self.d:
            kw["d_valid"] = self.d_valid
        return kw

    def _forward_pass(self, adj, Ys, F, *, perturbed, include_ego, batch_rows_only=False, need_last=False,
                      start_layer=0, noises=None, call_base=None):
        L = self.L
        x = self.E0 if start_layer == 0 else Ys[start_layer - 1]
        vf = self.vfree and adj is self.adj
        for k in range(start_layer, L):
            kw = {}
            if perturbed:
                noise = noises[k] if noises is not None else self._noise()
                call = self._noise_call if call_base is None else call_base + k
                kw.update(perturb_eps=self.eps, noise=noise, rng_seed=self.rng_seed, rng_offset=self._rng_offset(call),
                          rng_step=self.cursor[1:2] if noise is None else None,
                          rng_stride=self.P * self._rng_calls, **self._slice_kw())
                self._noise_call += 1
            if k == L - 1:
                prev = ([self.E0] if include_ego else []) + Ys[:L - 1]
                kw.update(prev=[self._loc(t) for t in prev], mean_div=float(L + 1 if include_ego else L),
                          mean_out=self._loc(F))
                if vf:
                    kw.update(prev_unscale=([False] if include_ego else []) + [True] * (L - 1))
                if batch_rows_only and self.use_marks:
                    kw.update(row_mark=self._loc(self.mark), mark_stamp=self.cursor[1:2])
            if vf:
                kw.update(row_scale=self.dinv, scale_in=k > 0, scale_out=k < L - 1)
            rider = {}
            if getattr(self, "_rider", None) is not None:
                rider, self._rider = {"fetch": self._rider}, None
            ops.spmm(adj, x, out=self._loc(Ys[k]), epilogue=ops.make_epilogue(**kw) if kw else None,
                     **({"pattern": True} if vf and k > 0 else {}), **rider)
            if k < L - 1 or need_last:
                self._allgather(Ys[k])
            x = Ys[k]
        self._allgather(F)

    def _simgcl_forward(self, adj):
        L, a, b = self.L, self.views[0], self.views[1]
        if L < 2:
            self._forward_pass(adj, self.Y, self.F, perturbed=False, include_ego=False, batch_rows_only=True)
            for v in (a, b):
                self._forward_pass(adj, v["Y"], v["F"], perturbed=True, include_ego=False, batch_rows_only=True)
            return
        na = [self._noise() for _ in range(L)] if self.noise_fn is not None else [None] * L
        nb = [self._noise() for _ in range(L)] if self.noise_fn is not None else [None] * L
        rider = {}
        if getattr(self, "_rider", None) is not None:
            rider, self._rider = {"fetch": self._rider}, None
        ops.spmm(adj, self.E0, out=self._loc(self.Y[0]), **rider, epilogue=ops.make_epilogue(
            perturb_eps=self.eps, noise=None, rng_seed=self.rng_seed, rng_offset=0,
            rng_step=self.cursor[1:2] if self.noise_fn is None else None, rng_stride=self.P * self._rng_calls, main_clean=True,
            **self._slice_kw(), **(dict(row_scale=self.dinv, scale_out=True) if self.vfree and adj is self.adj else {}),
            extra_out=[self._loc(a["Y"][0]), self._loc(b["Y"][0])], extra_noise=[na[0], nb[0]],
            extra_rng_offset=[self._rng_offset(0), self._rng_offset(L)]))
        for t in (self.Y[0], a["Y"][0], b["Y"][0]):
            self._allgather(t)
        self._forward_pass(adj, self.Y, self.F, perturbed=False, include_ego=False, batch_rows_only=True, start_layer=1)
# ... 77 lines not shown
                                            **{**sparse_add(add), **sparse_src, **skw, **akw}), **pkw)

    def _sparse_tables(self):
        clear = [self.gF] + [t for t in (self.gCL, self.gReg) if t is not None]
        if self.model == "SGL":
            clear += [v["gF"] for v in self.views]
        return clear

    def _step_before(self):
        self._step_front()
        if self.sync.active:
            self._step_grad()

    def _step_collective(self):
        self.colx.exchange()
        self.sync.reduce(self)

    def _step_after(self):
        if not self.sync.active:
            self._step_grad()
        self._step_opt()

    def _step_kernels(self):
        self._step_before()
        self._step_collective()
        self._step_after()

    def _sgl_shared_first(self):
        return self.model == "SGL" and self.L >= 2 and self.w == 64

    def _step_front(self):
        m, st = self.model, self.stage
        adj = self.adj
        cat = dict(stage_cat=self.stage_cat, n_cat=self.n_cat) if m == "SGL" else {}
        fetch = ((self._epoch_dev, self.sampler.n_edges, self.B, self.cursor, st, self.meta),
                 dict(row_mark=self.mark, mark_item_offset=0, zero4=self.losses, now=self.now,
                      half_batches=self.epoch_batches, **cat,
                      **(dict(adam_coef=self.adam_coef, adam_lr=self.lr) if self.fuse_adam else {})))
        self._rider = None
        if self.ride_fetch:
            self._rider = ops.batch_fetch_args(*fetch[0], **fetch[1])
        else:
            ops.batch_fetch(*fetch[0], **fetch[1])
        self._noise_call = 0

        include_ego = m in ("LightGCN", "SGL")
        sgl_shared_first = self._sgl_shared_first()
        if m == "SimGCL":
            self._simgcl_forward(adj)
        elif sgl_shared_first:
            a, b = self.views
            firsts = [self.Y[0], a["Y"][0], b["Y"][0]]
            ops.spmm3([adj, self.view_adj[0], self.view_adj[1]], self.E0, [self._loc(t) for t in firsts])
            for t in firsts:
                self._allgather(t)
            self._forward_pass(adj, self.Y, self.F, perturbed=False, include_ego=True, batch_rows_only=True, start_layer=1)
            for vi, v in enumerate(self.views):
                self._forward_pass(self.view_adj[vi], v["Y"], v["F"], perturbed=False, include_ego=True,
                                   batch_rows_only=True, start_layer=1)
        elif m != "MF":
            self._forward_pass(adj, self.Y, self.F, perturbed=(m == "XSimGCL"), include_ego=include_ego,
                               batch_rows_only=True, need_last=(m == "XSimGCL" and self.layer_cl == self.L))
        if m == "SGL" and not sgl_shared_first:
            for vi, v in enumerate(self.views):
                self._forward_pass(self.view_adj[vi], v["Y"], v["F"], perturbed=False, include_ego=include_ego,
                                   batch_rows_only=True)
        if self._rider is not None:
            raise SelfrecHipError("internal: the batch fetch found no product to ride on")
        self.colx.pack(self)

    def _step_back(self):
        self._step_grad()
        self.sync.reduce(self)
        self._step_opt()

    def _step_grad(self):
        m, st = self.model, self.stage
        adj = self.adj
        rows_dev, nuu_dev, nui_dev = self.meta[0:1], self.meta[1:2], self.meta[2:3]
        F = self.F
        T, GT, ix, cat_idx = self.colx.loss_views(self)
        if m == "LightGCN":
            reg_t, greg_t = self.E0, self.gReg
            reg_coef, inc_neg = self.reg / self.B, True
        elif m == "MF":
            reg_t, greg_t = F, self.gF
            reg_coef, inc_neg = self.reg / self.B, True
        else:
            reg_t, greg_t = F, self.gF
            reg_coef, inc_neg = self.reg, (m == "SGL")
        bpr = dict(batch=self.B, n_rows_dev=rows_dev, reg_coef=reg_coef, reg_include_neg=inc_neg, loss_scale=1.0,
                   g_user=GT(self.gF), g_item=GT(self.gF), greg_user=GT(greg_t), greg_item=GT(greg_t),
                   losses=self.losses[0:2])
        bpr_in = (T(F), T(F), T(reg_t), T(reg_t), ix["u"], ix["i"], ix["j"])
        seg = {}
        if self.det_scatter and not getattr(self, "_seg_off", False):
            ed = self._epoch_dev
            seg = dict(seg=dict(n_uniq_u=nuu_dev, n_uniq_i=nui_dev, n_uniq_n=ed["n_uniq_n"], seg_rows=ed["seg_rows"],
                                seg_end=ed["seg_end"], seg=ed["seg"], seg_a=ed["seg_a"], seg_b=ed["seg_b"],
                                batch_no=self.meta[3:4], rows_are_zero=self.sparse_reset))
        nce = dict(tau=self.tau, cl_scale=self.cl_rate, cl_loss=self.losses[2:3], nce_ws=self.nce_ws,
                   precision=self.nce_precision)
        if m == "XSimGCL":
            CL = self.E0 if self.layer_cl == 0 else self.Y[self.layer_cl - 1]
            ops.bpr_infonce(*bpr_in, **bpr, bpr_ws=self.bpr_ws, **nce, **seg, **({"nce_rows": 1} if seg else {}), problems=[
                (T(F), T(CL), ix["uniq_u"], self.B, nuu_dev, GT(self.gF), GT(self.gCL), True),
                (T(F), T(CL), ix["uniq_i"], self.B, nui_dev, GT(self.gF), GT(self.gCL), True)])
        elif m in ("SimGCL", "SGL"):
            a, b = self.views
            if m == "SimGCL":
                problems = [(T(a["F"]), T(b["F"]), ix["uniq_u"], self.B, nuu_dev, GT(self.gF), GT(self.gF)),
                            (T(a["F"]), T(b["F"]), ix["uniq_i"], self.B, nui_dev, GT(self.gF), GT(self.gF))]
            else:
                problems = [(T(a["F"]), T(b["F"]), cat_idx, 2 * self.B, self.n_cat, GT(a["gF"]), GT(b["gF"]))]
            ops.bpr_infonce(*bpr_in, **bpr, bpr_ws=self.bpr_ws, **nce, problems=problems, **seg,
                            **({"nce_rows": 1 if m == "SimGCL" else 2} if seg else {}))
        else:
            ops.bpr_l2_fwd_bwd(*bpr_in, **bpr, ws=self.bpr_ws, **seg)
        self.colx.scatter(self)
        if m == "MF":
            pass
        elif m == "XSimGCL":
            self._backward_chain(adj, self.gF, include_ego=False, gCL=self.gCL, layer_cl=self.layer_cl, final=True)
        elif m == "LightGCN":
            self._backward_chain(adj, self.gF, include_ego=True, extra=self.gReg, final=True)
        elif m == "SimGCL":
            self._backward_chain(adj, self.gF, include_ego=False, final=True)
        else:
            self._backward_chain(adj, self.gF, include_ego=True)
            for vi, v in enumerate(self.views):
                self._backward_chain(self.view_adj[vi], v["gF"], include_ego=True, accumulate=True,
                                     final=vi == len(self.views) - 1)

    def _step_opt(self):
        m, st = self.model, self.stage
        rows_dev, nuu_dev, nui_dev = self.meta[0:1], self.meta[1:2], self.meta[2:3]
        if self.fuse_adam:
            return
# ... 179 lines not shown
```

### selfrec_amd/ops.py

```python
from __future__ import annotations

import ctypes as C
import random as _pyrandom

import numpy as np
import torch

from . import _lib
from ._lib import SelfrecHipError, SpmmEpilogue, check

require_gpu = _lib.require_gpu


def gpu_available() -> bool:
    return torch.cuda.is_available()

__all__ = ["Sampler", "DeviceCSR", "column_class_order", "spmm", "spmm_any", "pad_cols", "padded_width", "spmm3", "spmm_probe", "spmm_set_xcd_shares", "spmm_plan_run_tasks", "adj_sym_normalize", "bpr_l2_fwd_bwd", "bpr_fwd", "bpr_bwd",
           "sumsq", "set_infonce_precision", "get_infonce_precision", "infonce_fwd_bwd", "infonce_multi", "bpr_infonce", "infonce_ws", "adam_step", "score_mask_topk", "score_mask_topk_filtered", "gemm_nt", "topk_rows", "topk_hit_flags", "metric_rows",
           "axpby", "batch_fetch", "zero_rows", "cursor_advance", "batch_lists", "batch_pack", "batch_unpack", "batch_scatter",
           "table_nce_ws", "table_nce_fwd_bwd", "kmeans_assign", "kmeans_update", "kmeans",
           "find_k_largest_host_f64", "knn_neighbours", "knn_score_ws", "knn_score_topk", "SelfrecHipError"]


def _stream() -> int:
# ... 235 lines not shown
                                             self.h_indptr.ctypes.data_as(C.c_void_p), int(split_len), int(xcd_split_row),
                                             None if h_mid is None else h_mid.ctypes.data_as(C.c_void_p)),
              "srh_spmm_plan_create")
        other._plan, other._plan_owner = h, None
        other.vals, other.nnz = self.vals, self.nnz
        other._arrays_of = self
        return other


def column_class_order(indptr, indices, min_len: int, bit: int = 0):
    indptr = np.asarray(indptr, dtype=np.int64)
    indices = np.asarray(indices)
    n = indptr.size - 1
    lens = np.diff(indptr)
    row_of = np.repeat(np.arange(n, dtype=np.int64), lens)
    odd = ((indices >> int(bit)) & 1).astype(np.int64)
    split = lens >= int(min_len)
    key = row_of * 2 + np.where(split[row_of], odd, 0)
    perm = np.argsort(key, kind="stable")
    n_odd = np.bincount(row_of, weights=odd, minlength=n).astype(np.int64)
    n_even = lens - n_odd
    row_mid = np.where(split, n_even, -1 - (n_odd > n_even).astype(np.int64)).astype(np.int32)
    return perm, row_mid


ADAM_EPILOGUE = True


def make_epilogue(*, perturb_eps=None, noise=None, rng_seed=0, rng_offset=0, rng_step=None,
                  rng_stride=0, prev=None, mean_div=None, mean_out=None, add=None, add_scale=None, alpha=1.0,
                  row_mark=None, col_mark=None, mark_stamp=None, add_mark=None, add_sparse=None,
                  extra_out=None, extra_noise=None, extra_rng_offset=None, main_clean=False, d_full=0, col0=0,
                  row_scale=None, scale_in=False, scale_out=False, prev_unscale=None, add_rowscale=None, d_valid=0,
                  adam=None):
    ep = SpmmEpilogue()
    if row_scale is not None:
        ep.d_row_scale = _p(row_scale, torch.float32, "row_scale")
        ep.scale_flags = (_lib.SRH_SCALE_IN if scale_in else 0) | (_lib.SRH_SCALE_OUT if scale_out else 0)
        ep.prev_unscale_mask = sum(1 << t for t, f in enumerate(prev_unscale or []) if f)
        ep.add_rowscale_mask = sum(1 << t for t, f in enumerate(add_rowscale or []) if f)
    ep.noise_d_full, ep.noise_col0 = int(d_full), int(col0)
    ep.noise_d_valid = int(d_valid)
    keep = []
    flags = 0
    if perturb_eps is not None:
        flags |= _lib.SRH_EPI_PERTURB
        ep.eps = float(perturb_eps)
        ep.d_noise = _p(noise, torch.float32, "noise")
        ep.rng_seed, ep.rng_offset = int(rng_seed), int(rng_offset)
        ep.d_rng_step = _p(rng_step, torch.int64, "rng_step")
        ep.rng_stride = int(rng_stride)
        keep += [noise, rng_step]
        extra_out = list(extra_out or [])
        if extra_out or main_clean:
            if len(extra_out) > _lib.SRH_MAX_EXTRA:
                raise SelfrecHipError(f"at most {_lib.SRH_MAX_EXTRA} extra perturbed outputs")
            ep.n_extra, ep.main_clean = len(extra_out), int(bool(main_clean))
            for k, t in enumerate(extra_out):
                ep.d_extra_out[k] = _p(t, torch.float32, "extra_out")
                ep.d_extra_noise[k] = _p((extra_noise or [None] * len(extra_out))[k], torch.float32, "extra_noise")
                ep.extra_rng_offset[k] = int((extra_rng_offset or [0] * len(extra_out))[k])
            keep += extra_out + list(extra_noise or [])
    if mean_out is not None:
        flags |= _lib.SRH_EPI_MEAN
        prev = list(prev or [])
        if len(prev) > _lib.SRH_MAX_PREV:
            raise SelfrecHipError(f"at most {_lib.SRH_MAX_PREV} earlier layers can be averaged in the epilogue")
# ... 8 lines not shown
        flags |= _lib.SRH_EPI_AXPY
        ep.alpha = float(alpha)
        if len(add) > _lib.SRH_MAX_ADD:
            raise SelfrecHipError(f"at most {_lib.SRH_MAX_ADD} addends")
        ep.n_add = len(add)
        for t, x in enumerate(add):
            ep.d_add[t] = _p(x, torch.float32, "add")
            ep.add_scale[t] = float(add_scale[t])
        keep += list(add)
    if row_mark is not None or col_mark is not None or add_mark is not None:
        ep.d_row_mark = _p(row_mark, torch.int32, "row_mark")
        ep.d_col_mark = _p(col_mark, torch.int32, "col_mark")
        ep.d_mark_stamp = _p(mark_stamp, torch.int64, "mark_stamp")
        ep.d_add_mark = _p(add_mark, torch.int32, "add_mark")
        ep.add_sparse_mask = sum(1 << t for t, f in enumerate(add_sparse or []) if f)
        keep += [row_mark, col_mark, mark_stamp, add_mark]
    if adam is not None:
        flags |= _lib.SRH_EPI_ADAM
        ep.d_adam_param, ep.d_adam_m, ep.d_adam_v = (_p(adam[k], torch.float32, k) for k in ("param", "m", "v"))
        ep.d_adam_coef = _p(adam["coef"], torch.float32, "coef")
        ep.adam_beta1, ep.adam_beta2 = float(adam.get("beta1", 0.9)), float(adam.get("beta2", 0.999))
        ep.adam_eps = float(adam.get("eps", 1e-8))
        clear = list(adam.get("clear") or [])
        if len(clear) > _lib.SRH_MAX_ADAM_CLEAR:
            raise SelfrecHipError(f"at most {_lib.SRH_MAX_ADAM_CLEAR} tables to clear")
        ep.adam_n_clear = len(clear)
        for k, t in enumerate(clear):
            ep.d_adam_clear[k] = _p(t, torch.float32, "clear")
        ep.d_adam_clear_mark = _p(adam.get("clear_mark"), torch.int32, "clear_mark")
        ep.d_adam_cursor = _p(adam.get("cursor"), torch.int64, "cursor")
        if mark_stamp is not None and not ep.d_mark_stamp:
            ep.d_mark_stamp = _p(mark_stamp, torch.int64, "mark_stamp")
        keep += [adam, mark_stamp]
    ep.flags = flags
    ep._keepalive = keep + [row_scale]
    return ep


def spmm(csr: DeviceCSR, x: torch.Tensor, out: torch.Tensor | None = None, epilogue: SpmmEpilogue | None = None,
         pattern: bool = False, fetch=None):
    if x.dim() != 2 or x.shape[0] != csr.shape[1]:
        raise SelfrecHipError(f"spmm: x has shape {tuple(x.shape)}, expected ({csr.shape[1]}, d)")
    d = int(x.shape[1])
    if out is None:
        out = torch.empty((csr.shape[0], d), dtype=torch.float32, device=x.device)
    common = (csr._plan, _p(csr.indptr, torch.int32), _p(csr.indices, torch.int32),
              None if pattern else _p(csr.vals, torch.float32, "vals"), _p(x, torch.float32, "x"),
              _p(out, torch.float32, "out"), d, C.byref(epilogue) if epilogue is not None else None)
    if fetch is not None:
        check(_lib.load().srh_spmm_f32_with_fetch(*common, C.byref(fetch), _stream()), "srh_spmm_f32_with_fetch")
    else:
        check(_lib.load().srh_spmm_f32(*common, _stream()), "srh_spmm_f32")
    return out


SPMM_WIDTHS = (8, 16, 32, 64, 128, 256)
ROW_WIDTHS = (32, 64, 128, 256)
NCE_WIDTHS = (64, 128, 256)


def padded_width(d: int, widths) -> int | None:
    return next((w for w in widths if w >= int(d)), None)


def pad_cols(t: torch.Tensor, width: int) -> torch.Tensor:
    d = int(t.shape[1])
# ... 235 lines not shown
    return torch.empty(int(_lib.load().srh_infonce_ws_bytes(n, d)), dtype=torch.uint8, device=device)


def infonce_fwd_bwd(v1, v2, idx, n, *, n_dev=None, tau, loss_scale, loss, g1, g2, ws):
    d = int(v1.shape[1])
    need = int(_lib.load().srh_infonce_ws_bytes(n, d))
    if ws.numel() * ws.element_size() < need:
        raise SelfrecHipError(f"infonce workspace too small: {ws.numel() * ws.element_size()} < {need}")
    check(_lib.load().srh_infonce_fwd_bwd(_p(v1, torch.float32), _p(v2, torch.float32), _p(idx, torch.int32), int(n),
                                          _p(n_dev, torch.int32), d, float(tau), float(loss_scale),
                                          _p(loss, torch.float64), _p(g1, torch.float32), _p(g2, torch.float32),
                                          _p(ws), _stream()), "srh_infonce_fwd_bwd")


def infonce_multi(problems, *, d, tau, loss_scale, loss, ws, precision=None):
    lib = _lib.load()
    arr = (_lib.InfonceProblem * len(problems))()
    need = 0
    for k, (v1, v2, idx, n, n_dev, g1, g2, *rest) in enumerate(problems):
        arr[k].d_v1, arr[k].d_v2 = _p(v1, torch.float32), _p(v2, torch.float32)
        arr[k].d_idx, arr[k].n, arr[k].d_n = _p(idx, torch.int32), int(n), _p(n_dev, torch.int32)
        arr[k].d_g1, arr[k].d_g2 = _p(g1, torch.float32), _p(g2, torch.float32)
        arr[k].g2_exclusive = int(bool(rest[0])) if rest else 0
        need += int(lib.srh_infonce_ws_bytes(n, d))
    if ws.numel() * ws.element_size() < need:
        raise SelfrecHipError(f"infonce workspace too small: {ws.numel() * ws.element_size()} < {need}")
    check(lib.srh_infonce_fwd_bwd_multi(arr, len(problems), int(d), float(tau), float(loss_scale),
                                        _p(loss, torch.float64), _p(ws), _nce_mode(precision), _stream()),
          "srh_infonce_fwd_bwd_multi")


def bpr_infonce(user, item, reg_user, reg_item, u_idx, i_idx, j_idx, *, batch, n_rows_dev=None, reg_coef,
                reg_include_neg, loss_scale, g_user, g_item, greg_user, greg_item, losses, bpr_ws,
                problems, tau, cl_scale, cl_loss, nce_ws, precision=None, seg=None, nce_rows=0):
    lib = _lib.load()
    d = int(user.shape[1])
    b = _bpr_problem(user, item, reg_user, reg_item, u_idx, i_idx, j_idx, batch, n_rows_dev, reg_coef, reg_include_neg,
                     loss_scale, g_user, g_item, greg_user, greg_item, losses, bpr_ws, seg, nce_rows)
    arr = (_lib.InfonceProblem * len(problems))()
    need = 0
    for k, (v1, v2, idx, n, n_dev, g1, g2, *rest) in enumerate(problems):
        arr[k].d_v1, arr[k].d_v2 = _p(v1, torch.float32), _p(v2, torch.float32)
        arr[k].d_idx, arr[k].n, arr[k].d_n = _p(idx, torch.int32), int(n), _p(n_dev, torch.int32)
        arr[k].d_g1, arr[k].d_g2 = _p(g1, torch.float32), _p(g2, torch.float32)
        arr[k].g2_exclusive = int(bool(rest[0])) if rest else 0
        need += int(lib.srh_infonce_ws_bytes(n, d))
    if nce_ws.numel() * nce_ws.element_size() < need:
        raise SelfrecHipError(f"infonce workspace too small: {nce_ws.numel() * nce_ws.element_size()} < {need}")
    check(lib.srh_bpr_infonce_fwd_bwd(C.byref(b), arr, len(problems), d, float(tau), float(cl_scale),
                                      _p(cl_loss, torch.float64), _p(nce_ws), _nce_mode(precision), _stream()),
          "srh_bpr_infonce_fwd_bwd")


def adam_step(param, grad, m, v, *, step=0, step_dev=None, lr, beta1=0.9, beta2=0.999, eps=1e-8, clear=None,
              row_mark=None, advance_cursor=None):
    if clear is not None or advance_cursor is not None:
        clear = list(clear or [])
        tables = (C.c_void_p * max(1, len(clear)))(*[_p(t, torch.float32, "clear") for t in clear])
        check(_lib.load().srh_adam_step_reset(_p(param, torch.float32), _p(grad, torch.float32), _p(m, torch.float32),
                                              _p(v, torch.float32), int(param.shape[0]), int(param.shape[1]),
                                              _p(step_dev, torch.int64), float(lr), float(beta1), float(beta2), float(eps),
                                              _p(row_mark, torch.int32), len(clear), tables,
                                              _p(advance_cursor, torch.int64), _stream()), "srh_adam_step_reset")
        return
    check(_lib.load().srh_adam_step(_p(param, torch.float32), _p(grad, torch.float32), _p(m, torch.float32),
                                    _p(v, torch.float32), param.numel(), int(step), _p(step_dev, torch.int64),
                                    float(lr), float(beta1), float(beta2), float(eps), _stream()), "srh_adam_step")


def score_mask_topk(user_emb, user_ids, item_emb, r_indptr, r_indices, k, scores_ws=None):
    nq = int(user_ids.numel()) if user_ids is not None else int(user_emb.shape[0])
# ... 87 lines not shown
    hits = torch.empty((len(cuts), n), dtype=torch.int32, device=dev)
    ndcg = torch.empty((len(cuts), n), dtype=torch.float64, device=dev)
    arr = (C.c_int32 * len(cuts))(*cuts)
    check(_lib.load().srh_metric_rows(_p(flags, torch.uint8), _p(sizes, torch.int32), n, k, arr, len(cuts),
                                      _p(d_gains, torch.float64), _p(d_ideal, torch.float64), _p(hits, torch.int32),
                                      _p(ndcg, torch.float64), _stream()), "srh_metric_rows")
    return hits, ndcg


def axpby(a, x, b, y):
    check(_lib.load().srh_axpby(float(a), _p(x, torch.float32), float(b), _p(y, torch.float32), x.numel(), _stream()),
          "srh_axpby")
    return y


def cursor_advance(cursor):
    check(_lib.load().srh_cursor_advance(_p(cursor, torch.int64), _stream()), "srh_cursor_advance")


def zero_rows(lists, d, cursor_advance=None):
    n = len(lists)
    vp = C.c_void_p * n
    tables = vp(*[_p(t, torch.float32, "table") for t, *_ in lists])
    idx = vp(*[_p(i, torch.int32, "idx") for _, i, *_ in lists])
    cnt = vp(*[_p(c, torch.int32, "count") for _, _, c, *_ in lists])
    n_max = (C.c_int32 * n)(*[int(m) for *_, m, _ in lists])
    off = (C.c_int32 * n)(*[int(o) for *_, o in lists])
    check(_lib.load().srh_zero_rows(n, tables, idx, cnt, n_max, off, int(d), _p(cursor_advance, torch.int64),
                                    _stream()), "srh_zero_rows")


def batch_fetch_args(ep, n_edges, batch_size, cursor, stage, meta, row_mark=None, mark_item_offset=0, zero4=None,
                     stage_cat=None, cat_item_offset=0, n_cat=None, now=None, half_batches=0, adam_coef=None, adam_lr=0.0,
                     adam_beta1=0.9, adam_beta2=0.999):
    a = _lib.BatchFetchArgs()
    a.d_epoch_u, a.d_epoch_i, a.d_epoch_j = (_p(ep[k], torch.int32) for k in ("u", "i", "j"))
    a.d_epoch_uniq_u, a.d_epoch_uniq_i = _p(ep.get("uniq_u"), torch.int32), _p(ep.get("uniq_i"), torch.int32)
    a.d_n_uniq_u, a.d_n_uniq_i = _p(ep.get("n_uniq_u"), torch.int32), _p(ep.get("n_uniq_i"), torch.int32)
    a.n_edges, a.batch_size, a.d_cursor = int(n_edges), int(batch_size), _p(cursor, torch.int64)
    a.d_stage_u, a.d_stage_i, a.d_stage_j = (_p(stage[k], torch.int32) for k in ("u", "i", "j"))
    a.d_stage_uniq_u, a.d_stage_uniq_i = _p(stage.get("uniq_u"), torch.int32), _p(stage.get("uniq_i"), torch.int32)
    a.d_meta, a.d_row_mark = _p(meta, torch.int32), _p(row_mark, torch.int32)
    a.mark_item_offset, a.cat_item_offset = int(mark_item_offset), int(cat_item_offset)
    a.d_zero4, a.d_stage_cat, a.d_n_cat = _p(zero4, torch.float64), _p(stage_cat, torch.int32), _p(n_cat, torch.int32)
    a.d_now = _p(now, torch.int64)
    a.half_batches = int(half_batches)
    a.d_adam_coef = _p(adam_coef, torch.float32)
    a.adam_lr, a.adam_beta1, a.adam_beta2 = float(adam_lr), float(adam_beta1), float(adam_beta2)
    a._keepalive = [ep, cursor, stage, meta, row_mark, zero4, stage_cat, n_cat, now, adam_coef]
    return a


def batch_fetch(*args, **kwargs):
    a = args[0] if len(args) == 1 and isinstance(args[0], _lib.BatchFetchArgs) else batch_fetch_args(*args, **kwargs)
    check(_lib.load().srh_batch_fetch(C.byref(a), _stream()), "srh_batch_fetch")


def batch_lists(stage, meta, batch_size):
    bl = _lib.BatchLists()
    keep = []
    for s, (name, cnt) in enumerate((("u", 0), ("i", 0), ("j", 0), ("uniq_u", 1), ("uniq_i", 2))):
        c = meta[cnt:cnt + 1]
        bl.d_idx[s] = _p(stage[name], torch.int32, name)
        bl.d_count[s] = _p(c, torch.int32, "count")
        keep += [stage[name], c]
    bl.B = int(batch_size)
    bl._keepalive = keep
    return bl


def _ptr_array(tensors, name):
    return (C.c_void_p * len(tensors))(*[_p(t, torch.float32, name) for t in tensors])


def batch_pack(lists, tables, send, cat_idx=None, n_cat=None):
    dl = int(tables[0].shape[1])
    rows = 5 * lists.B
    if send.numel() < len(tables) * rows * dl or any(int(t.shape[1]) != dl for t in tables):
        raise SelfrecHipError("batch_pack: send buffer too small / tables of different widths")
    check(_lib.load().srh_batch_pack(C.byref(lists), len(tables), _ptr_array(tables, "table"), dl,
                                     _p(send, torch.float32, "send"), _p(cat_idx, torch.int32, "cat_idx"),
                                     _p(n_cat, torch.int32, "n_cat"), _stream()), "srh_batch_pack")
# ... 219 lines not shown
```

Measured before the change: 7.079 million pairs/s.

## Fuse InfoNCE prep into SpMM epilogue and BPR phase1 into NCE pass1

Batch fetch now writes a per-row map (stamp, unique index) for the batch's unique users and items. The SpMM epilogue uses that map to write the normalized NCE view rows and norms directly into the InfoNCE workspace, and the BPR phase-1 reduction rides on extra blocks at the tail of the first f32 NCE tile pass. Together these drop the separate nce_prep_bpr1 launch and the re-read of embeddings it needed. The cost is more epilogue work and register pressure in the SpMM kernel, a larger NCE tile grid, and a new map table. The fused path is only used for single-GPU XSimGCL with d=64 and all-f32 NCE.

```diff
diff --git a/include/selfrec_hip.h b/include/selfrec_hip.h
--- a/include/selfrec_hip.h
+++ b/include/selfrec_hip.h
@@ -74,7 +74,7 @@
 int32_t srh_spmm_plan_run_tasks(const srh_spmm_plan_t* plan, int32_t d);
 void srh_spmm_plan_destroy(srh_spmm_plan_t* plan);
 
-enum { SRH_EPI_PERTURB = 1, SRH_EPI_MEAN = 2, SRH_EPI_AXPY = 4, SRH_EPI_ADAM = 8 };
+enum { SRH_EPI_PERTURB = 1, SRH_EPI_MEAN = 2, SRH_EPI_AXPY = 4, SRH_EPI_ADAM = 8, SRH_EPI_NCE_PREP = 16 };
 #define SRH_MAX_ADAM_CLEAR 4
 #define SRH_MAX_PREV 8
 #define SRH_MAX_ADD 2
@@ -122,6 +122,12 @@
   const int32_t* d_adam_clear_mark;
   float* d_adam_clear[SRH_MAX_ADAM_CLEAR];
   int64_t* d_adam_cursor;
+  const int32_t* d_nce_map;
+  void* d_nce_ws;
+  int64_t nce_n_max[2];
+  const int32_t* d_nce_n[2];
+  int32_t nce_count;
+  int32_t nce_view2;
 } srh_spmm_epilogue_t;
 enum { SRH_SCALE_IN = 1, SRH_SCALE_OUT = 2 };
 
@@ -221,6 +227,7 @@
   double* d_losses;
   void* d_ws;
   const srh_batch_segments_t* seg;
+  int32_t nce_prepared;
 } srh_bpr_problem_t;
 srh_status_t srh_bpr_l2_fwd_bwd_p(const srh_bpr_problem_t* bpr, int32_t d, void* stream);
 srh_status_t srh_bpr_infonce_fwd_bwd(const srh_bpr_problem_t* bpr, const srh_infonce_problem_t* problems,
@@ -290,6 +297,7 @@
   int64_t half_batches;
   float* d_adam_coef;
   float adam_lr, adam_beta1, adam_beta2;
+  int32_t* d_nce_map;
 } srh_batch_fetch_args_t;
 srh_status_t srh_batch_fetch(const srh_batch_fetch_args_t* args, void* stream);
 srh_status_t srh_spmm_f32_with_fetch(const srh_spmm_plan_t* plan, const int32_t* d_indptr, const int32_t* d_indices,
diff --git a/selfrec_amd/_lib.py b/selfrec_amd/_lib.py
--- a/selfrec_amd/_lib.py
+++ b/selfrec_amd/_lib.py
@@ -9,7 +9,7 @@
 LIB_PATH = os.path.join(_HERE, "lib", "libselfrec_hip.so")
 ABI_VERSION = 31
 
-SRH_EPI_PERTURB, SRH_EPI_MEAN, SRH_EPI_AXPY, SRH_EPI_ADAM = 1, 2, 4, 8
+SRH_EPI_PERTURB, SRH_EPI_MEAN, SRH_EPI_AXPY, SRH_EPI_ADAM, SRH_EPI_NCE_PREP = 1, 2, 4, 8, 16
 SRH_MAX_ADAM_CLEAR = 4
 SRH_SCALE_IN, SRH_SCALE_OUT = 1, 2
 SRH_MAX_PREV, SRH_MAX_ADD, SRH_MAX_EXTRA = 8, 2, 2
@@ -28,7 +28,7 @@
                 ("d_row_mark", C.c_void_p), ("mark_item_offset", C.c_int32), ("cat_item_offset", C.c_int32),
                 ("d_zero4", C.c_void_p), ("d_stage_cat", C.c_void_p), ("d_n_cat", C.c_void_p), ("d_now", C.c_void_p),
                 ("half_batches", C.c_int64), ("d_adam_coef", C.c_void_p), ("adam_lr", C.c_float),
-                ("adam_beta1", C.c_float), ("adam_beta2", C.c_float)]
+                ("adam_beta1", C.c_float), ("adam_beta2", C.c_float), ("d_nce_map", C.c_void_p)]
 
 
 class InfonceProblem(C.Structure):
@@ -60,7 +60,7 @@
                 ("d_n_rows", C.c_void_p), ("reg_coef", C.c_float), ("reg_include_neg", C.c_int32),
                 ("loss_scale", C.c_float), ("d_g_user", C.c_void_p), ("d_g_item", C.c_void_p),
                 ("d_greg_user", C.c_void_p), ("d_greg_item", C.c_void_p), ("d_losses", C.c_void_p), ("d_ws", C.c_void_p),
-                ("seg", C.POINTER(BatchSegments))]
+                ("seg", C.POINTER(BatchSegments)), ("nce_prepared", C.c_int32)]
 
 
 class SpmmEpilogue(C.Structure):
@@ -84,6 +84,8 @@
         ("d_adam_param", C.c_void_p), ("d_adam_m", C.c_void_p), ("d_adam_v", C.c_void_p), ("d_adam_coef", C.c_void_p),
         ("adam_beta1", C.c_float), ("adam_beta2", C.c_float), ("adam_eps", C.c_float), ("adam_n_clear", C.c_int32),
         ("d_adam_clear_mark", C.c_void_p), ("d_adam_clear", C.c_void_p * SRH_MAX_ADAM_CLEAR), ("d_adam_cursor", C.c_void_p),
+        ("d_nce_map", C.c_void_p), ("d_nce_ws", C.c_void_p), ("nce_n_max", C.c_int64 * 2), ("d_nce_n", C.c_void_p * 2),
+        ("nce_count", C.c_int32), ("nce_view2", C.c_int32),
     ]
 
 
diff --git a/selfrec_amd/csrc/common.h b/selfrec_amd/csrc/common.h
--- a/selfrec_amd/csrc/common.h
+++ b/selfrec_amd/csrc/common.h
@@ -79,6 +79,11 @@
     f.d_adam_coef[0] = (float)((double)f.adam_lr / (1.0 - pow((double)f.adam_beta1, t)));
     f.d_adam_coef[1] = (float)sqrt(1.0 - pow((double)f.adam_beta2, t));
   }
+  if (f.d_nce_map && f.d_epoch_uniq_u && rows > 0) {
+    int2* map = reinterpret_cast<int2*>(f.d_nce_map);
+    for (int64_t i = tid; i < a; i += nth) map[f.d_epoch_uniq_u[b * bs + i]] = make_int2(stamp, (int32_t)i);
+    for (int64_t i = tid; i < c; i += nth) map[f.d_epoch_uniq_i[b * bs + i]] = make_int2(stamp, (1 << 24) | (int32_t)i);
+  }
   if (tid == 0) {
     f.d_meta[0] = (int32_t)rows;
     f.d_meta[1] = a;
@@ -86,6 +91,63 @@
     f.d_meta[3] = (int32_t)b;
   }
 }
+
+constexpr int kNceSplits = 16;
+constexpr int kNceMaxProblems = 4;
+constexpr int kNceQueryBlock = 128, kNceKeyBlock = 32, kNceMaxPer = 128;
+constexpr unsigned long long kLossUnreported = ~0ull;
+__host__ __device__ inline int64_t nce_pad(int64_t n) { return (n + 63) / 64 * 64; }
+
+struct NcePlan {
+  int n[kNceMaxProblems], per[kNceMaxProblems], splits[kNceMaxProblems], first[kNceMaxProblems + 1];
+};
+__device__ __forceinline__ void nce_plan_cut(const int (&n_in)[kNceMaxProblems], const int slots, NcePlan& p) {
+  int qb[kNceMaxProblems], kb[kNceMaxProblems];
+  int t_min = 1;
+  long long work = 0;
+#pragma unroll
+  for (int k = 0; k < kNceMaxProblems; ++k) {
+    const int n = n_in[k];
+    p.n[k] = n;
+    const int np = (int)nce_pad(n);
+    qb[k] = (np + kNceQueryBlock - 1) / kNceQueryBlock;
+    kb[k] = np / kNceKeyBlock;
+    t_min = max(t_min, (kb[k] + kNceSplits - 1) / kNceSplits);
+    work += (long long)qb[k] * kb[k];
+  }
+  int t = max(t_min, (int)((work + slots - 1) / slots));
+  int best_t = t;
+  long long best_cost = -1;
+  for (int it = 0; it < 32; ++it, ++t) {
+    int tasks = 0;
+#pragma unroll
+    for (int k = 0; k < kNceMaxProblems; ++k) tasks += qb[k] * ((kb[k] + t - 1) / t);
+    const int rounds = (tasks + slots - 1) / slots;
+    const long long cost = (long long)rounds * t;
+    if (best_cost < 0 || cost < best_cost) { best_cost = cost; best_t = t; }
+    if (rounds <= 1) break;
+  }
+  p.first[0] = 0;
+#pragma unroll
+  for (int k = 0; k < kNceMaxProblems; ++k) {
+    const int sp = kb[k] > 0 ? (kb[k] + best_t - 1) / best_t : 0;
+    p.splits[k] = sp;
+    p.per[k] = sp > 0 ? (kb[k] + sp - 1) / sp : 0;
+    p.first[k + 1] = p.first[k] + qb[k] * sp;
+  }
+}
+
+struct NcePrepFuse {
+  const int2* map;
+  int count, view2, slots;
+  float *v1n[2], *v2n[2], *norm1[2], *norm2[2];
+  int32_t* ticket[2];
+  unsigned long long* losspart[2];
+  NcePlan* plan;
+  const int32_t* d_n[2];
+  int n_max[2], np[2];
+};
+srh_status_t nce_prep_fuse_args(void* ws, const int64_t* n_max, const int32_t* const* d_n, int count, int d, NcePrepFuse& out);
 
 __device__ __forceinline__ float4 f4_zero() { return make_float4(0.f, 0.f, 0.f, 0.f); }
 template <bool WT>
diff --git a/selfrec_amd/csrc/losses.hip b/selfrec_amd/csrc/losses.hip
--- a/selfrec_amd/csrc/losses.hip
+++ b/selfrec_amd/csrc/losses.hip
@@ -40,12 +40,14 @@
   int n_blocks;
 };
 
-template <int LPR>
-__device__ __forceinline__ void bpr_phase1_body(const BprArgs& a, const unsigned block_id) {
+template <int LPR, int HALVES = 1>
+__device__ __forceinline__ void bpr_phase1_body(const BprArgs& a, unsigned block_id) {
   constexpr int G = 64 / LPR;
   const int rows = a.d_n_rows ? min(*a.d_n_rows, a.B) : a.B;
   const int lane = threadIdx.x & 63, g = lane / LPR, sub = lane % LPR;
-  const int b = (int)((block_id * 256u + threadIdx.x) >> 6) * G + g;
+  const unsigned t256 = threadIdx.x & 255u;
+  if (HALVES > 1) block_id += threadIdx.x >> 8;
+  const int b = (int)((block_id * 256u + t256) >> 6) * G + g;
   const bool valid = b < rows;
   const int bu = valid ? a.u_idx[b] : 0, bi = valid ? a.i_idx[b] : 0, bj = valid ? a.j_idx[b] : 0;
   const float4 u = reinterpret_cast<const float4*>(a.user)[(size_t)bu * LPR + sub];
@@ -66,17 +68,17 @@
   double su = valid ? (double)f4_dot(ru, ru) : 0.0;
   double sp = valid ? (double)f4_dot(rp, rp) : 0.0;
   double sn = valid ? (double)f4_dot(rn, rn) : 0.0;
-  __shared__ double s_part[4][4];
+  __shared__ double s_part[4 * HALVES][4];
   l_part = wave_sum_d(l_part);
   su = wave_sum_d(su);
   sp = wave_sum_d(sp);
   sn = wave_sum_d(sn);
-  const int wv = threadIdx.x >> 6;
+  const int wv = threadIdx.x >> 6, w0 = (wv >> 2) * 4;
   if (lane == 0) { s_part[wv][0] = l_part; s_part[wv][1] = su; s_part[wv][2] = sp; s_part[wv][3] = sn; }
   __syncthreads();
-  if (threadIdx.x < 4)
-    a.part[(size_t)block_id * 4 + threadIdx.x] =
-        s_part[0][threadIdx.x] + s_part[1][threadIdx.x] + s_part[2][threadIdx.x] + s_part[3][threadIdx.x];
+  if (t256 < 4 && (HALVES == 1 || (int)block_id < a.n_blocks))
+    a.part[(size_t)block_id * 4 + t256] =
+        s_part[w0][t256] + s_part[w0 + 1][t256] + s_part[w0 + 2][t256] + s_part[w0 + 3][t256];
 }
 
 template <int LPR>
@@ -256,7 +258,6 @@
   for (int64_t i = (int64_t)wg * 256 + threadIdx.x; i < n; i += stride) g[i] = x[i] * coef;
 }
 
-constexpr int kNceSplits = 16;
 constexpr float kNceKqScale = 32.0f;
 constexpr float kNceInvKqScale2 = 1.0f / (kNceKqScale * kNceKqScale);
 #ifndef SRH_NCE_SPLITS
@@ -276,7 +277,6 @@
 
 std::atomic<int> g_nce_precision{getenv("SRH_NCE_SPLIT16") ? SRH_NCE_SPLIT16 : SRH_NCE_F32};
 
-constexpr unsigned long long kLossUnreported = ~0ull;
 
 struct NceWs {
   float *v1n, *v2n, *norm1, *norm2, *opart, *opart2, *lpart, *invl;
@@ -294,7 +294,6 @@
   float *g1, *g2;
   int g2_plain;
 };
-constexpr int kNceMaxProblems = 4;
 struct NceBatch {
   NceWs w[kNceMaxProblems];
   int count;
@@ -303,50 +302,15 @@
   int f32_only;
 };
 
-__host__ __device__ inline int64_t nce_pad(int64_t n) { return (n + 63) / 64 * 64; }
-
-struct NcePlan {
-  int n[kNceMaxProblems], per[kNceMaxProblems], splits[kNceMaxProblems], first[kNceMaxProblems + 1];
-};
-constexpr int kNceQueryBlock = 128, kNceKeyBlock = 32, kNceMaxPer = 128;
 constexpr int kNceReuseMax = 8192;
 
 
 __device__ __forceinline__ void nce_plan(const NceBatch& b, NcePlan& p) {
-  int qb[kNceMaxProblems], kb[kNceMaxProblems];
-  int t_min = 1;
-  long long work = 0;
-#pragma unroll
-  for (int k = 0; k < kNceMaxProblems; ++k) {
-    int n = 0;
-    if (k < b.count) n = max(0, b.w[k].d_n ? min(*b.w[k].d_n, b.w[k].n_max) : b.w[k].n_max);
-    p.n[k] = n;
-    const int np = (int)nce_pad(n);
-    qb[k] = (np + kNceQueryBlock - 1) / kNceQueryBlock;
-    kb[k] = np / kNceKeyBlock;
-    t_min = max(t_min, (kb[k] + kNceSplits - 1) / kNceSplits);
-    work += (long long)qb[k] * kb[k];
-  }
-  int t = max(t_min, (int)((work + b.slots - 1) / b.slots));
-  int best_t = t;
-  long long best_cost = -1;
-  for (int it = 0; it < 32; ++it, ++t) {
-    int tasks = 0;
-#pragma unroll
-    for (int k = 0; k < kNceMaxProblems; ++k) tasks += qb[k] * ((kb[k] + t - 1) / t);
-    const int rounds = (tasks + b.slots - 1) / b.slots;
-    const long long cost = (long long)rounds * t;
-    if (best_cost < 0 || cost < best_cost) { best_cost = cost; best_t = t; }
-    if (rounds <= 1) break;
-  }
-  p.first[0] = 0;
-#pragma unroll
-  for (int k = 0; k < kNceMaxProblems; ++k) {
-    const int sp = kb[k] > 0 ? (kb[k] + best_t - 1) / best_t : 0;
-    p.splits[k] = sp;
-    p.per[k] = sp > 0 ? (kb[k] + sp - 1) / sp : 0;
-    p.first[k + 1] = p.first[k] + qb[k] * sp;
-  }
+  int n[kNceMaxProblems];
+#pragma unroll
+  for (int k = 0; k < kNceMaxProblems; ++k)
+    n[k] = k < b.count ? max(0, b.w[k].d_n ? min(*b.w[k].d_n, b.w[k].n_max) : b.w[k].n_max) : 0;
+  nce_plan_cut(n, b.slots, p);
 }
 
 
@@ -810,7 +774,7 @@
 }
 
 template <int D, bool PASS2, bool REUSE>
-__global__ __launch_bounds__(512) void nce_tile_f32(NceBatch batch, float inv_tau) {
+__global__ __launch_bounds__(512) void nce_tile_f32(NceBatch batch, float inv_tau, BprArgs bpr, int n_bpr) {
   constexpr int DQ = D / 4;
   constexpr int NT = D / 16;
   constexpr int NV = NT / 4;
@@ -1127,6 +1091,10 @@
       if (g == 0) const_cast<float*>(lpart)[(size_t)split * stride + qrow] = lsum;
     }
     SRH_STAMP(4);
+  }
+  if (!PASS2 && n_bpr > 0) {
+    const int j = (int)blockIdx.x - ((int)gridDim.x - (n_bpr + 1) / 2);
+    if (j >= 0) bpr_phase1_body<D / 4, 2>(bpr, 2u * (unsigned)j);
   }
 }
 
@@ -1398,7 +1366,7 @@
 template <int D>
 srh_status_t launch_infonce(const srh_infonce_problem_t* pr, int count, float tau, float loss_scale, double* loss,
                             void* ws, hipStream_t st, int precision, const BprArgs* bpr = nullptr,
-                            const SegArgs* seg = nullptr) {
+                            const SegArgs* seg = nullptr, bool prepared = false) {
   constexpr int LPR = D / 4, G = 64 / LPR;
   NceBatch batch{};
   batch.count = count;
@@ -1440,11 +1408,19 @@
   if (bpr) {
     bp = *bpr;
     n_bpr = bp.n_blocks = ((bp.B + G - 1) / G + 3) / 4;
+  }
+  int n_bpr_pass1 = 0;
+  if (prepared) {
+    SRH_REQUIRE(bpr && f32 && D == 64 && count <= 2 && grid_f32 > 0 && 2 * grid_f32 >= n_bpr,
+                "bpr_infonce_fwd_bwd: nce_prepared needs the BPR problem, the all-f32 passes, d = 64 and <= 2 problems");
+    n_bpr_pass1 = n_bpr;
+  } else if (bpr) {
     nce_prep_bpr1<LPR><<<n_bpr + (int)(gp.x * 2 * count), 256, 0, st>>>(batch, bp, n_bpr, (int)gp.x);
+    SRH_LAUNCH_CHECK();
   } else {
     nce_prep<LPR><<<gp, 256, 0, st>>>(batch);
-  }
-  SRH_LAUNCH_CHECK();
+    SRH_LAUNCH_CHECK();
+  }
   NceFinishArgs fa{inv_tau, loss_scale, loss};
   dim3 fb((np_max / G + 3) / 4, 1, count);
   if (!f32) {
@@ -1473,13 +1449,13 @@
     bool reuse = true;
     for (int k = 0; k < count; ++k) reuse = reuse && batch.w[k].etile != nullptr;
     if (reuse) {
-      nce_tile_f32<D, false, true><<<grid_f32, 512, kLds, st>>>(batch, inv_tau);
+      nce_tile_f32<D, false, true><<<grid_f32, 512, kLds, st>>>(batch, inv_tau, bp, n_bpr_pass1);
       SRH_LAUNCH_CHECK();
-      nce_tile_f32<D, true, true><<<grid_f32, 512, kLds, st>>>(batch, inv_tau);
+      nce_tile_f32<D, true, true><<<grid_f32, 512, kLds, st>>>(batch, inv_tau, bp, 0);
     } else {
-      nce_tile_f32<D, false, false><<<grid_f32, 512, kLds, st>>>(batch, inv_tau);
+      nce_tile_f32<D, false, false><<<grid_f32, 512, kLds, st>>>(batch, inv_tau, bp, n_bpr_pass1);
       SRH_LAUNCH_CHECK();
-      nce_tile_f32<D, true, false><<<grid_f32, 512, kLds, st>>>(batch, inv_tau);
+      nce_tile_f32<D, true, false><<<grid_f32, 512, kLds, st>>>(batch, inv_tau, bp, 0);
     }
     SRH_LAUNCH_CHECK();
   }
@@ -1647,7 +1623,7 @@
 
 static srh_status_t infonce_entry(const srh_infonce_problem_t* problems, int32_t n_problems, int32_t d, float tau,
                                   float loss_scale, double* d_loss, void* d_ws, int32_t precision, void* stream,
-                                  const BprArgs* bpr, const SegArgs* seg = nullptr) {
+                                  const BprArgs* bpr, const SegArgs* seg = nullptr, bool prepared = false) {
   SRH_REQUIRE(precision == SRH_NCE_DEFAULT || precision == SRH_NCE_SPLIT16 || precision == SRH_NCE_F32,
               "infonce_fwd_bwd: unknown precision %d", precision);
   if (precision == SRH_NCE_DEFAULT) {
@@ -1675,10 +1651,37 @@
     return SRH_ERR_UNSUPPORTED;
   }
   hipStream_t st = srh::as_stream(stream);
-  if (d == 64) return launch_infonce<64>(problems, n_problems, tau, loss_scale, d_loss, d_ws, st, precision, bpr, seg);
+  SRH_REQUIRE(!prepared || precision == SRH_NCE_F32, "bpr_infonce_fwd_bwd: nce_prepared serves the all-f32 passes only");
+  if (d == 64) return launch_infonce<64>(problems, n_problems, tau, loss_scale, d_loss, d_ws, st, precision, bpr, seg, prepared);
   if (d == 128) return launch_infonce<128>(problems, n_problems, tau, loss_scale, d_loss, d_ws, st, precision, bpr, seg);
   return launch_infonce<256>(problems, n_problems, tau, loss_scale, d_loss, d_ws, st, precision, bpr, seg);
 }
+
+}
+
+srh_status_t srh::nce_prep_fuse_args(void* ws, const int64_t* n_max, const int32_t* const* d_n, int count, int d,
+                                     NcePrepFuse& out) {
+  SRH_REQUIRE(ws && count >= 1 && count <= 2, "nce_prep: 1 or 2 problems and a workspace");
+  out = NcePrepFuse{};
+  out.count = count;
+  out.slots = srh::cu_count();
+  char* cursor = reinterpret_cast<char*>(ws);
+  for (int k = 0; k < count; ++k) {
+    SRH_REQUIRE(n_max[k] > 0 && n_max[k] < (int64_t(1) << 24), "nce_prep: bad n in problem %d", k);
+    const NceWs w = carve_nce(cursor, n_max[k], d);
+    cursor += srh_infonce_ws_bytes(n_max[k], d);
+    out.v1n[k] = w.v1n; out.v2n[k] = w.v2n; out.norm1[k] = w.norm1; out.norm2[k] = w.norm2;
+    out.ticket[k] = w.ticket;
+    out.losspart[k] = reinterpret_cast<unsigned long long*>(w.losspart);
+    if (k == 0) out.plan = w.plan;
+    out.d_n[k] = d_n[k];
+    out.n_max[k] = (int)n_max[k];
+    out.np[k] = (int)w.np;
+  }
+  return SRH_OK;
+}
+
+extern "C" {
 
 #ifdef SRH_NCEF32_STAMPS
 srh_status_t srh_debug_nce_stamps(unsigned long long* h_out ) {
@@ -1717,7 +1720,8 @@
   SegArgs sg{};
   if (b->seg)
     if (srh_status_t st = seg_args(b->seg, n_problems, sg)) return st;
-  return infonce_entry(problems, n_problems, d, tau, cl_scale, d_cl_loss, d_nce_ws, precision, stream, &a, b->seg ? &sg : nullptr);
+  return infonce_entry(problems, n_problems, d, tau, cl_scale, d_cl_loss, d_nce_ws, precision, stream, &a, b->seg ? &sg : nullptr,
+                       b->nce_prepared != 0);
 }
 
 srh_status_t srh_bpr_l2_fwd_bwd_p(const srh_bpr_problem_t* b, int32_t d, void* stream) {
diff --git a/selfrec_amd/csrc/spmm.hip b/selfrec_amd/csrc/spmm.hip
--- a/selfrec_amd/csrc/spmm.hip
+++ b/selfrec_amd/csrc/spmm.hip
@@ -56,6 +56,7 @@
   const int32_t* adam_clear_mark;
   float4* adam_clear[SRH_MAX_ADAM_CLEAR];
   int64_t* adam_cursor;
+  NcePrepFuse nce;
 };
 
 __device__ __forceinline__ uint32_t lowbias32(uint32_t x) {
@@ -142,11 +143,23 @@
   return y;
 }
 
-template <int LPR, bool ADAM = false>
+template <int LPR>
+__device__ __forceinline__ void nce_put_view(float4 v, int i, int sub, float* __restrict__ out, float* __restrict__ nrm) {
+  const float ss = group_sum<LPR>(f4_dot(v, v));
+  const float norm = sqrtf(ss);
+  const float den = fmaxf(norm, 1e-12f);
+  const float4 o = make_float4(v.x / den, v.y / den, v.z / den, v.w / den);
+  reinterpret_cast<float4*>(out)[(size_t)i * LPR + sub] = o;
+  if (sub == 0) nrm[i] = norm;
+}
+
+template <int LPR, bool ADAM = false, bool NCE = false>
 __device__ __forceinline__ void row_epilogue(float4 y, int row, int sub, bool store, float4* __restrict__ Y,
                                              const DevEpilogue& ep, const float r = 1.0f) {
   if (!store) return;
   const size_t at = (size_t)row * LPR + sub;
+  int2 nce_at = make_int2(0, 0);
+  if constexpr (NCE) nce_at = ep.nce.map[row];
   float4 mm, vv, pp;
   if constexpr (ADAM) {
     mm = ep.adam_m[at]; vv = ep.adam_v[at]; pp = ep.adam_p[at];
@@ -183,15 +196,19 @@
       if (store) st_f4<kYWT>(reinterpret_cast<float4*>(ep.extra_out[k]) + at, out_scaled ? f4_scale(yk, r) : yk);
     }
   }
-  if (store) st_f4<kYWT>(Y + at, out_scaled ? f4_scale(y, r) : y);
+  const float4 y_stored = out_scaled ? f4_scale(y, r) : y;
+  if (store) st_f4<kYWT>(Y + at, y_stored);
   if (ep.flags & SRH_EPI_MEAN) {
     const float rinv = (ep.prev_unscale && r > 0.f) ? 1.0f / r : 0.f;
     float4 m = y;
+    float4 view2 = y_stored;
     if (ep.n_prev > 0) {
       m = reinterpret_cast<const float4*>(ep.prev[0])[at];
+      if (NCE && ep.nce.view2 == 0) view2 = m;
       if (ep.prev_unscale & 1) m = f4_scale(m, rinv);
       for (int t = 1; t < ep.n_prev; ++t) {
         float4 pt = reinterpret_cast<const float4*>(ep.prev[t])[at];
+        if (NCE && ep.nce.view2 == t) view2 = pt;
         if ((ep.prev_unscale >> t) & 1) pt = f4_scale(pt, rinv);
         m = f4_add(m, pt);
       }
@@ -200,7 +217,43 @@
     if (store) {
       float4 o = f4_scale(m, ep.mean_rcp);
       st_f4<kYWT>(reinterpret_cast<float4*>(ep.mean_out) + at, o);
-    }
+      if constexpr (NCE) {
+        const int k = nce_at.y >> 24, i = nce_at.y & 0xffffff;
+        if (nce_at.x == (int)(*ep.mark_stamp) && k < ep.nce.count) {
+          const bool one = k != 0;
+          nce_put_view<LPR>(o, i, sub, one ? ep.nce.v1n[1] : ep.nce.v1n[0], one ? ep.nce.norm1[1] : ep.nce.norm1[0]);
+          nce_put_view<LPR>(view2, i, sub, one ? ep.nce.v2n[1] : ep.nce.v2n[0], one ? ep.nce.norm2[1] : ep.nce.norm2[0]);
+        }
+      }
+    }
+  }
+}
+
+template <int LPR>
+__device__ __forceinline__ void nce_side_body(const NcePrepFuse& f, const int block, const int n_blocks) {
+  const int tid = block * 256 + (int)threadIdx.x, nth = n_blocks * 256;
+  int n[kNceMaxProblems] = {0, 0, 0, 0};
+#pragma unroll
+  for (int k = 0; k < 2; ++k) {
+    if (k >= f.count) break;
+    const int np = f.np[k];
+    n[k] = f.d_n[k] ? min(*f.d_n[k], f.n_max[k]) : f.n_max[k];
+    for (int j = tid; j <= np / 16; j += nth) f.ticket[k][j] = 0;
+    for (int j = tid; j < np; j += nth) f.losspart[k][j] = kLossUnreported;
+    const int lo = max(n[k], 0);
+    for (int q = tid; q < (np - lo) * LPR; q += nth) {
+      const int i = lo + q / LPR, sub = q % LPR;
+      reinterpret_cast<float4*>(f.v1n[k])[(size_t)i * LPR + sub] = f4_zero();
+      reinterpret_cast<float4*>(f.v2n[k])[(size_t)i * LPR + sub] = f4_zero();
+      if (sub == 0) { f.norm1[k][i] = 0.f; f.norm2[k][i] = 0.f; }
+    }
+  }
+  if (tid == 0) {
+#pragma unroll
+    for (int k = 0; k < kNceMaxProblems; ++k) n[k] = max(0, n[k]);
+    NcePlan plan;
+    nce_plan_cut(n, f.slots, plan);
+    *f.plan = plan;
   }
 }
 
@@ -351,7 +404,8 @@
   int32_t row[4], start[4], end[4];
 };
 
-template <int LPR, bool COLMASK, bool PROBE = false, bool LATEPF = false, bool FLOOR = false, bool ADAM = false>
+template <int LPR, bool COLMASK, bool PROBE = false, bool LATEPF = false, bool FLOOR = false, bool ADAM = false,
+          bool NCE = false>
 __global__ __launch_bounds__(256) __attribute__((amdgpu_waves_per_eu(8, 8))) void spmm_rows_kernel(const Task64* __restrict__ tasks, int n_tasks,
                                                         const int32_t* __restrict__ indices,
                                                         const float* __restrict__ vals,
@@ -364,7 +418,8 @@
   constexpr int G = 64 / LPR;
   constexpr int CH = 16 * G;
   if ((int)blockIdx.x < n_fetch) {
-    srh::batch_fetch_body(rider, (int)blockIdx.x, n_fetch);
+    if constexpr (NCE) nce_side_body<LPR>(ep.nce, (int)blockIdx.x, n_fetch);
+    else srh::batch_fetch_body(rider, (int)blockIdx.x, n_fetch);
     return;
   }
   const int wave = __builtin_amdgcn_readfirstlane((int)(((blockIdx.x - n_fetch) * 256u + threadIdx.x) >> 6));
@@ -492,7 +547,7 @@
 #pragma unroll
     for (int m = LPR; m < 64; m <<= 1) a4 = f4_add(a4, f4_shfl_xor(a4, m));
     if (slot < 0) {
-      row_epilogue<LPR, ADAM>(a4, row, sub, g == 0, Y, ep, r);
+      row_epilogue<LPR, ADAM, NCE>(a4, row, sub, g == 0, Y, ep, r);
       leave();
       return;
     }
@@ -510,7 +565,7 @@
     float4 sum = sum_partials_agent(partial + (size_t)hfirst * LPR + sub, g, G, hn, LPR);
 #pragma unroll
     for (int m = LPR; m < 64; m <<= 1) sum = f4_add(sum, f4_shfl_xor(sum, m));
-    row_epilogue<LPR, ADAM>(sum, row, sub, g == 0, Y, ep, r);
+    row_epilogue<LPR, ADAM, NCE>(sum, row, sub, g == 0, Y, ep, r);
     leave();
     return;
   }
@@ -538,7 +593,7 @@
     const float4 a4 = total();
     if (a4.x == 123456.789f) Y[0] = a4;
   } else {
-    row_epilogue<LPR, ADAM>(total(), row, sub, live, Y, ep, r);
+    row_epilogue<LPR, ADAM, NCE>(total(), row, sub, live, Y, ep, r);
   }
   leave();
 }
@@ -1101,7 +1156,7 @@
 static srh_status_t translate_epilogue(const srh_spmm_epilogue_t* epi, int32_t d, const float* d_x, const float* d_y,
                                        DevEpilogue& ep) {
   if (epi) {
-    SRH_REQUIRE((epi->flags & ~(SRH_EPI_PERTURB | SRH_EPI_MEAN | SRH_EPI_AXPY | SRH_EPI_ADAM)) == 0,
+    SRH_REQUIRE((epi->flags & ~(SRH_EPI_PERTURB | SRH_EPI_MEAN | SRH_EPI_AXPY | SRH_EPI_ADAM | SRH_EPI_NCE_PREP)) == 0,
                 "spmm_f32: unknown epilogue flag");
     ep.flags = epi->flags;
     ep.eps = epi->eps;
@@ -1192,6 +1247,18 @@
       ep.adam_clear[k] = reinterpret_cast<float4*>(epi->d_adam_clear[k]);
     }
     ep.adam_cursor = epi->d_adam_cursor;
+  }
+  if (epi && (epi->flags & SRH_EPI_NCE_PREP)) {
+    SRH_REQUIRE(d == 64 && (epi->flags & SRH_EPI_MEAN) && epi->d_row_mark && !epi->d_col_mark && !epi->noise_d_full,
+                "spmm_f32: NCE_PREP rides on a row-masked MEAN launch over whole rows of 64 columns");
+    SRH_REQUIRE(epi->nce_count >= 1 && epi->nce_count <= 2 && epi->d_nce_map && epi->d_nce_ws,
+                "spmm_f32: NCE_PREP needs 1 or 2 problems, the row map and the InfoNCE workspace");
+    SRH_REQUIRE(epi->nce_view2 >= -1 && epi->nce_view2 < epi->n_prev, "spmm_f32: NCE_PREP: nce_view2 %d outside [-1, %d)",
+                epi->nce_view2, epi->n_prev);
+    if (srh_status_t rc = srh::nce_prep_fuse_args(epi->d_nce_ws, epi->nce_n_max, epi->d_nce_n, epi->nce_count, d, ep.nce))
+      return rc;
+    ep.nce.map = reinterpret_cast<const int2*>(epi->d_nce_map);
+    ep.nce.view2 = epi->nce_view2;
   }
   if (!ep.noise_d_full) { ep.noise_d_full = d; ep.noise_col0 = 0; }
   ep.noise_d_valid = ep.noise_d_full;
@@ -1504,6 +1571,7 @@
     if (srh_status_t rc = srh::check_fetch_args(fetch, fetch_args)) return rc;
     n_fetch = srh::kFetchBlocks;
   }
+  SRH_REQUIRE(!(fetch && epi && (epi->flags & SRH_EPI_NCE_PREP)), "spmm_f32_with_fetch: no NCE_PREP on the fetch launch");
   SRH_REQUIRE(plan && d_indices && d_x && d_y, "spmm_f32: null argument");
   SRH_REQUIRE(d_vals || (d >= 64 && !(epi && epi->d_col_mark)),
               "spmm_f32: a pattern matrix (d_vals == NULL) needs d >= 64 and no column marks");
@@ -1551,6 +1619,9 @@
         if (d == 64) SRH_LAUNCH_ROWS(16, 1, false, false, false, false, true);
         else if (d == 128) SRH_LAUNCH_ROWS(32, 2, false, false, false, false, true);
         else SRH_LAUNCH_ROWS(64, 3, false, false, false, false, true);
+      } else if (ep.row_mark && d == 64 && (ep.flags & SRH_EPI_NCE_PREP)) {
+        n_fetch = srh::kFetchBlocks;
+        SRH_LAUNCH_ROWS(16, 1, false, false, true, false, false, true);
       } else if (ep.row_mark && d == 64) {
         SRH_LAUNCH_ROWS(16, 1, false, false, true);
       } else {
diff --git a/selfrec_amd/engine.py b/selfrec_amd/engine.py
--- a/selfrec_amd/engine.py
+++ b/selfrec_amd/engine.py
@@ -7,7 +7,7 @@
 import torch
 import torch.distributed as _dist
 
-from . import layouts, ops
+from . import _lib, layouts, ops
 from ._lib import SelfrecHipError
 from .comm import AbiComm, TorchComm, TwoHopRows, default_comm, shard_adjacency
 from .layouts import SLICE_WIDTHS, parse_grid
@@ -145,6 +145,10 @@
         if model in ("XSimGCL", "SimGCL", "SGL"):
             one = ops.infonce_ws(2 * B if model == "SGL" else B, d, dev)
             self.nce_ws = torch.empty(one.numel() * (1 if model == "SGL" else 2), dtype=torch.uint8, device=dev)
+        self.fuse_nce_prep = (single and model == "XSimGCL" and self.w == 64 and 1 <= self.layer_cl <= self.L
+                              and not self.colx.split and os.environ.get("SRH_FUSED_NCE_PREP", "1") != "0")
+        self.nce_map = torch.zeros((P, 2), dtype=torch.int32, device=dev) if self.fuse_nce_prep else None
+        self._nce_fused_now = False
         E = self.sampler.n_edges
         self.epoch_batches = (E + B - 1) // B
         nb = self.epoch_batches
@@ -415,8 +419,16 @@
             kw["d_valid"] = self.d_valid
         return kw
 
+    def _nce_fused(self):
+        if not self.fuse_nce_prep:
+            return False
+        mode = ops._nce_mode(self.nce_precision)
+        if mode == ops.NCE_DEFAULT:
+            mode = int(_lib.load().srh_infonce_get_precision())
+        return mode == ops.NCE_PRECISIONS["f32"]
+
     def _forward_pass(self, adj, Ys, F, *, perturbed, include_ego, batch_rows_only=False, need_last=False,
-                      start_layer=0, noises=None, call_base=None):
+                      start_layer=0, noises=None, call_base=None, nce_prep=None):
         L = self.L
         x = self.E0 if start_layer == 0 else Ys[start_layer - 1]
         vf = self.vfree and adj is self.adj
@@ -437,6 +449,8 @@
                     kw.update(prev_unscale=([False] if include_ego else []) + [True] * (L - 1))
                 if batch_rows_only and self.use_marks:
                     kw.update(row_mark=self._loc(self.mark), mark_stamp=self.cursor[1:2])
+                    if nce_prep is not None:
+                        kw.update(nce_prep=nce_prep)
             if vf:
                 kw.update(row_scale=self.dinv, scale_in=k > 0, scale_out=k < L - 1)
             rider = {}
@@ -580,11 +594,13 @@
     def _step_front(self):
         m, st = self.model, self.stage
         adj = self.adj
+        self._nce_fused_now = self._nce_fused()
         cat = dict(stage_cat=self.stage_cat, n_cat=self.n_cat) if m == "SGL" else {}
         fetch = ((self._epoch_dev, self.sampler.n_edges, self.B, self.cursor, st, self.meta),
                  dict(row_mark=self.mark, mark_item_offset=0, zero4=self.losses, now=self.now,
                       half_batches=self.epoch_batches, **cat,
-                      **(dict(adam_coef=self.adam_coef, adam_lr=self.lr) if self.fuse_adam else {})))
+                      **(dict(adam_coef=self.adam_coef, adam_lr=self.lr) if self.fuse_adam else {}),
+                      **(dict(nce_map=self.nce_map) if self._nce_fused_now else {})))
         self._rider = None
         if self.ride_fetch:
             self._rider = ops.batch_fetch_args(*fetch[0], **fetch[1])
@@ -607,8 +623,12 @@
                 self._forward_pass(self.view_adj[vi], v["Y"], v["F"], perturbed=False, include_ego=True,
                                    batch_rows_only=True, start_layer=1)
         elif m != "MF":
+            nce_prep = None
+            if self._nce_fused_now:
+                nce_prep = dict(map=self.nce_map, ws=self.nce_ws, n_max=[self.B, self.B], n_dev=[self.meta[1:2], self.meta[2:3]],
+                                view2=self.layer_cl - 1 if self.layer_cl < self.L else -1)
             self._forward_pass(adj, self.Y, self.F, perturbed=(m == "XSimGCL"), include_ego=include_ego,
-                               batch_rows_only=True, need_last=(m == "XSimGCL" and self.layer_cl == self.L))
+                               batch_rows_only=True, need_last=(m == "XSimGCL" and self.layer_cl == self.L), nce_prep=nce_prep)
         if m == "SGL" and not sgl_shared_first:
             for vi, v in enumerate(self.views):
                 self._forward_pass(self.view_adj[vi], v["Y"], v["F"], perturbed=False, include_ego=include_ego,
@@ -651,7 +671,8 @@
                    precision=self.nce_precision)
         if m == "XSimGCL":
             CL = self.E0 if self.layer_cl == 0 else self.Y[self.layer_cl - 1]
-            ops.bpr_infonce(*bpr_in, **bpr, bpr_ws=self.bpr_ws, **nce, **seg, **({"nce_rows": 1} if seg else {}), problems=[
+            ops.bpr_infonce(*bpr_in, **bpr, bpr_ws=self.bpr_ws, **nce, **seg, **({"nce_rows": 1} if seg else {}),
+                            **({"nce_prepared": True} if self._nce_fused_now else {}), problems=[
                 (T(F), T(CL), ix["uniq_u"], self.B, nuu_dev, GT(self.gF), GT(self.gCL), True),
                 (T(F), T(CL), ix["uniq_i"], self.B, nui_dev, GT(self.gF), GT(self.gCL), True)])
         elif m in ("SimGCL", "SGL"):
diff --git a/selfrec_amd/ops.py b/selfrec_amd/ops.py
--- a/selfrec_amd/ops.py
+++ b/selfrec_amd/ops.py
@@ -291,7 +291,7 @@
                   row_mark=None, col_mark=None, mark_stamp=None, add_mark=None, add_sparse=None,
                   extra_out=None, extra_noise=None, extra_rng_offset=None, main_clean=False, d_full=0, col0=0,
                   row_scale=None, scale_in=False, scale_out=False, prev_unscale=None, add_rowscale=None, d_valid=0,
-                  adam=None):
+                  adam=None, nce_prep=None):
     ep = SpmmEpilogue()
     if row_scale is not None:
         ep.d_row_scale = _p(row_scale, torch.float32, "row_scale")
@@ -366,6 +366,15 @@
         if mark_stamp is not None and not ep.d_mark_stamp:
             ep.d_mark_stamp = _p(mark_stamp, torch.int64, "mark_stamp")
         keep += [adam, mark_stamp]
+    if nce_prep is not None:
+        flags |= _lib.SRH_EPI_NCE_PREP
+        n_max, n_dev = list(nce_prep["n_max"]), list(nce_prep["n_dev"])
+        ep.d_nce_map = _p(nce_prep["map"], torch.int32, "nce map")
+        ep.d_nce_ws = _p(nce_prep["ws"])
+        ep.nce_count, ep.nce_view2 = len(n_max), int(nce_prep["view2"])
+        for k in range(len(n_max)):
+            ep.nce_n_max[k], ep.d_nce_n[k] = int(n_max[k]), _p(n_dev[k], torch.int32, "n")
+        keep += [nce_prep]
     ep.flags = flags
     ep._keepalive = keep + [row_scale]
     return ep
@@ -667,11 +676,12 @@
 
 def bpr_infonce(user, item, reg_user, reg_item, u_idx, i_idx, j_idx, *, batch, n_rows_dev=None, reg_coef,
                 reg_include_neg, loss_scale, g_user, g_item, greg_user, greg_item, losses, bpr_ws,
-                problems, tau, cl_scale, cl_loss, nce_ws, precision=None, seg=None, nce_rows=0):
+                problems, tau, cl_scale, cl_loss, nce_ws, precision=None, seg=None, nce_rows=0, nce_prepared=False):
     lib = _lib.load()
     d = int(user.shape[1])
     b = _bpr_problem(user, item, reg_user, reg_item, u_idx, i_idx, j_idx, batch, n_rows_dev, reg_coef, reg_include_neg,
                      loss_scale, g_user, g_item, greg_user, greg_item, losses, bpr_ws, seg, nce_rows)
+    b.nce_prepared = int(bool(nce_prepared))
     arr = (_lib.InfonceProblem * len(problems))()
     need = 0
     for k, (v1, v2, idx, n, n_dev, g1, g2, *rest) in enumerate(problems):
@@ -825,7 +835,7 @@
 
 def batch_fetch_args(ep, n_edges, batch_size, cursor, stage, meta, row_mark=None, mark_item_offset=0, zero4=None,
                      stage_cat=None, cat_item_offset=0, n_cat=None, now=None, half_batches=0, adam_coef=None, adam_lr=0.0,
-                     adam_beta1=0.9, adam_beta2=0.999):
+                     adam_beta1=0.9, adam_beta2=0.999, nce_map=None):
     a = _lib.BatchFetchArgs()
     a.d_epoch_u, a.d_epoch_i, a.d_epoch_j = (_p(ep[k], torch.int32) for k in ("u", "i", "j"))
     a.d_epoch_uniq_u, a.d_epoch_uniq_i = _p(ep.get("uniq_u"), torch.int32), _p(ep.get("uniq_i"), torch.int32)
@@ -840,7 +850,8 @@
     a.half_batches = int(half_batches)
     a.d_adam_coef = _p(adam_coef, torch.float32)
     a.adam_lr, a.adam_beta1, a.adam_beta2 = float(adam_lr), float(adam_beta1), float(adam_beta2)
-    a._keepalive = [ep, cursor, stage, meta, row_mark, zero4, stage_cat, n_cat, now, adam_coef]
+    a.d_nce_map = _p(nce_map, torch.int32, "nce_map")
+    a._keepalive = [ep, cursor, stage, meta, row_mark, zero4, stage_cat, n_cat, now, adam_coef, nce_map]
     return a
 
 
```

Measured after the change: 7.110 million pairs/s (median of 6 runs). No clear change (+0.4%).
